# marella/ctransformers

Measured on NVIDIA H100. Metric: decode tokens/s Llama-2-7B Q4_K_M b=1, higher is better.
Workload: dtype int8 (q4_K/q6_K weights x q8_K activations, mma.sync u8 x s8 -> exact int32), fp32 combine in the reference's order

## Files before the change

ctransformers_b200/csrc/engine.cu:

```cuda
#include "engine.cuh"

#include <algorithm>
#include <chrono>
#include <cstdio>
#include <cstring>
#include <stdexcept>

#include "attention.cuh"
#include "matvec.cuh"
#include "prefill.cuh"
#include "repack.cuh"
#include "sample_gpu.cuh"
#include "score_gpu.cuh"
#include "stream.cuh"
#include "tables.hpp"
#include "tp_nccl.hpp"

namespace ctb {

#define CTB_CUDA(expr)                                                                                         \
  do {                                                                                                         \
    cudaError_t e__ = (expr);                                                                                  \
    if (e__ != cudaSuccess)                                                                                    \
      throw std::runtime_error(std::string("CUDA error: ") + cudaGetErrorString(e__) + " at " + __FILE__ + ":" + \
// ... 467 lines not shown
  };
  auto take_input = [&](MVParams& p) {
    if (!xchg_due) return;
    p.x = (const float*)xc_ll_[tp_.rank]; p.x_mode = 2; p.x_parts = tp_.world; p.x_stride = n_embd; p.sum_out = x_sum_into;
  };
  auto mark_exchange = [&](size_t first_op) {
    if (!xchg_due) return;
    if (ops_.size() != first_op + 1) throw std::runtime_error("tensor parallel (fused exchange): the consumer of an exchange must be one mat-vec phase");
    fill_xc(ops_[first_op].ph.xc, 1);
    n_xchg++;
    xchg_due = false; x_sum_into = nullptr;
  };
  const float kq_scale = 1.0f / sqrtf((float)n_embd / (float)hp_.n_head);
  ops_.clear();
  {
    StepOp op{};
    op.ph.kind = PH_EMBED;
    op.ph.em.table = tok_embd_; op.ph.em.row_bytes = tok_row_bytes_; op.ph.em.tokens = d_state_; op.ph.em.out = xa_;
    op.ph.em.type = tok_type_; op.ph.em.K = n_embd; op.ph.em.n_vocab = hp_.n_vocab;
    ops_.push_back(op);
  }
  float* x = xa_;
  float* y = xb_;
  for (int il = 0; il < hp_.n_layer; il++) {
    const LayerW& L = layers_[il];
    uint16_t* kc = kc_ + (size_t)il * hp_.n_ctx * n_kv * k_stride(hd);
    uint16_t* vc = vc_ + (size_t)il * gqa * kv_ctx_pad(hp_.n_ctx);
    AttnParams ap{};
    ap.kc = kc; ap.vc = vc; ap.out = attn_; ap.exp_tab = exp_tab_; ap.state = d_state_; ap.kq_scale = kq_scale;
    ap.n_head = nh_; ap.n_kv = n_kv; ap.hd = hd; ap.n_ctx = hp_.n_ctx; ap.rope = rope_; ap.neox = hp_.falcon ? 1 : 0;
    auto push_attn = [&]() {
      StepOp op{};
      op.ph.kind = PH_ATTN;
      op.ph.at = ap;
      ops_.push_back(op);
    };

    if (!hp_.falcon) {
      float* q = qkv_; float* k = qkv_ + qw; float* v = qkv_ + qw + gqa;
      {
        MVParams p{};
        p.x = x; p.norm_w = L.attn_norm; p.norm_mode = NORM_RMS; p.eps = hp_.eps; p.K = n_embd;
        const size_t first_op = ops_.size();
        take_input(p);
        const DevMat* ws[3] = {&L.wq, &L.wk, &L.wv};
        float* outs[3] = {q, k, v};
        bool done[3] = {false, false, false};
        ap.q = q; ap.k = k; ap.v = v; ap.q_stride = qw; ap.kv_stride = gqa;
        for (int i = 0; i < 3; i++) {
          if (done[i]) continue;
          p.act = act_format_for(ws[i]->type); p.nseg = 0;
          for (int j = i; j < 3; j++)
            if (!done[j] && act_format_for(ws[j]->type) == p.act) { p.seg[p.nseg++] = seg(*ws[j], outs[j]); done[j] = true; }
          push_matvec(p, MVK_QKV);
        }
        mark_exchange(first_op);
      }
      push_attn();
      {
        MVParams p{};
        p.x = attn_; p.norm_mode = NORM_NONE; p.K = qw; p.act = act_format_for(L.wo.type); p.nseg = 1;
        p.seg[0] = (!tp || tp_lead) ? seg(L.wo, y, EPI_ADD, x) : seg(L.wo, y);
        push_matvec(p, MVK_WO);
        if (tp) push_xchg(y);
      }
      {
        MVParams p{};
        p.x = y; p.norm_w = L.ffn_norm; p.norm_mode = NORM_RMS; p.eps = hp_.eps; p.K = n_embd;
        const size_t first_op = ops_.size();
        take_input(p);
        p.act = act_format_for(L.w1.type); p.nseg = 2;
        p.seg[0] = seg(L.w1, ffn_, EPI_SILU); p.seg[1] = seg(L.w3, ffn2_);
        push_matvec(p, MVK_UP);
        mark_exchange(first_op);
      }
      {
        MVParams p{};
        p.x = ffn_; p.x2 = ffn2_; p.x_mode = 1; p.norm_mode = NORM_NONE; p.K = nff_; p.act = act_format_for(L.w2.type); p.nseg = 1;
        p.seg[0] = (!tp || tp_lead) ? seg(L.w2, x, EPI_ADD, y) : seg(L.w2, x);
        push_matvec(p, MVK_DOWN);
        if (tp) push_xchg(x);
      }
    } else {
      const int qkv_w = (hp_.n_head + 2 * n_kv) * hd;
      float* q = qkv_; float* k = qkv_ + (size_t)hp_.n_head * hd; float* v = k + (size_t)n_kv * hd;
      const bool two_norms = L.attn_norm2 != nullptr;
      const bool fuse = !two_norms && act_format_for(L.wqkv.type) == act_format_for(L.w3.type);
      {
        MVParams p{};
        p.x = x; p.norm_mode = NORM_LAYER; p.eps = hp_.eps; p.K = n_embd;
        p.norm_w = two_norms ? L.attn_norm2 : L.attn_norm; p.norm_b = two_norms ? L.attn_norm2_b : L.attn_norm_b;
        p.act = act_format_for(L.wqkv.type); p.nseg = 1;
        p.seg[0] = seg(L.wqkv, qkv_);
        if (fuse) { p.seg[1] = seg(L.w3, ffn_, EPI_GELU); p.nseg = 2; }
        ap.q = q; ap.k = k; ap.v = v; ap.q_stride = qkv_w; ap.kv_stride = qkv_w;
        push_matvec(p, MVK_QKV);
      }
      if (!fuse) {
        MVParams p{};
        p.x = x; p.norm_mode = NORM_LAYER; p.eps = hp_.eps; p.K = n_embd; p.norm_w = L.attn_norm; p.norm_b = L.attn_norm_b;
        p.act = act_format_for(L.w3.type); p.nseg = 1;
        p.seg[0] = seg(L.w3, ffn_, EPI_GELU);
        push_matvec(p, MVK_UP);
      }
      push_attn();
      {
        MVParams p{};
        p.x = attn_; p.norm_mode = NORM_NONE; p.K = n_embd; p.act = act_format_for(L.wo.type); p.nseg = 1;
        p.seg[0] = seg(L.wo, attn_o_);
        push_matvec(p, MVK_WO);
      }
      {
        MVParams p{};
        p.x = ffn_; p.norm_mode = NORM_NONE; p.K = hp_.n_ff; p.act = act_format_for(L.w2.type); p.nseg = 1;
        p.seg[0] = seg(L.w2, y, EPI_ADD2, attn_o_, x);
        push_matvec(p, MVK_DOWN);
      }
      std::swap(x, y);
    }
  }
  n_body_ = (int)ops_.size();
  {
    MVParams p{};
    p.x = x; p.norm_w = out_norm_; p.norm_b = out_norm_b_; p.norm_mode = hp_.falcon ? NORM_LAYER : NORM_RMS; p.eps = hp_.eps; p.K = n_embd;
    const size_t first_op = ops_.size();
    take_input(p);
    p.norm_out = d_embd_; p.act = act_format_for(output_.type); p.nseg = 1;
    p.seg[0] = seg(output_, d_logits_);
    push_matvec(p, MVK_OUT);
    mark_exchange(first_op);

  }
  {
    StepOp op{};
    op.ph.kind = PH_PICK;
    op.ph.pk.logits = d_logits_; op.ph.pk.state = d_state_; op.ph.pk.out_tokens = nullptr; op.ph.pk.n = hp_.n_vocab;
    ops_.push_back(op);
  }
  bool any_stream = false;
  for (const StepOp& op : ops_) any_stream |= op.ph.kind == PH_MATVEC && op.stream;
  std::vector<Phase> phs;
  for (const StepOp& op : ops_) if (op.ph.kind != PH_XCHG && (op.ph.kind != PH_MATVEC || op.stream)) phs.push_back(op.ph);
  const StepLaunch sl = step_launch_shape(phs.data(), (int)phs.size(), sm_count_, max_dyn_smem(k_step<true, false, false>));
  step_grid_ = sl.grid; step_slots_ = sl.n_slots; step_smem_ = sl.smem; step_q3_ = sl.q3;
  if (const char* e = getenv("CTB_ST_SLOTS")) {
    const int want = atoi(e);
    if (want >= ST_W && want < step_slots_ && want % ST_W == 0) { step_smem_ -= (size_t)(step_slots_ - want) * ST_SLOT; step_slots_ = want; }
  }
  ring_attn_ = st_attn_ring_ok(hp_.n_ctx, step_slots_) && !getenv("CTB_NO_RING_ATTN");
  for (StepOp& op : ops_) if (op.ph.kind == PH_ATTN) op.ph.q6 = ring_attn_ ? 1 : 0;
  if (any_stream && step_slots_ < ST_W) throw std::runtime_error("model rows are too long for the step kernel's shared memory");
  if (any_stream) CTB_CUDA(step_set_smem_limit(step_smem_));
  else fused_ = false;
  d_prog_ = (Phase*)alloc((ops_.size() + 1) * sizeof(Phase), 256);
  d_prog_mv_ = (Phase*)alloc((ops_.size() + 1) * sizeof(Phase), 256);
  d_bounds_ = (int*)alloc((ops_.size() + 1) * (size_t)(sm_count_ + 1) * 4, 256);
  d_bounds_mv_ = (int*)alloc((ops_.size() + 1) * (size_t)(sm_count_ + 1) * 4, 256);
}

void Engine::upload_prog(Phase* dst, int* dst_bounds, const std::vector<StepOp>& ops) {
  std::vector<Phase> phs(ops.size());
  for (size_t i = 0; i < ops.size(); i++) phs[i] = ops[i].ph;
  CTB_CUDA(cudaMemcpy(dst, phs.data(), phs.size() * sizeof(Phase), cudaMemcpyHostToDevice));
  std::vector<Phase> run = phs;
  for (size_t i = 0; i < ops.size(); i++) if (ops[i].ph.kind == PH_XCHG || (ops[i].ph.kind == PH_MATVEC && !ops[i].stream)) run[i].kind = -1;
  const std::vector<int> b = step_bounds(run.data(), (int)run.size(), sm_count_);
  CTB_CUDA(cudaMemcpy(dst_bounds, b.data(), b.size() * 4, cudaMemcpyHostToDevice));
}

struct ProfMark {
  Event ev;
  int kind;
};

long Engine::enqueue_ops(const std::vector<StepOp>& ops, const Phase* d_prog, const int* d_bounds, int n, cudaStream_t st, bool fused,
                         std::vector<ProfMark>* marks) {
  long launches = 0;
  auto mark = [&](int kind) {
    if (!marks) return;
    marks->push_back({Event(cudaEventDefault), kind});
    CTB_CUDA(cudaEventRecord(marks->back().ev, st));
  };
  StepLaunch step_shape_;
  step_shape_.grid = step_grid_; step_shape_.n_slots = step_slots_; step_shape_.smem = step_smem_; step_shape_.gen = !attn_fast_hd(hp_.head_dim());
  step_shape_.q3 = step_q3_;
  auto capable = [&](const StepOp& op) { return op.ph.kind != PH_XCHG && (op.ph.kind != PH_MATVEC || op.stream); };
  int i = 0;
  while (i < n) {
    const StepOp& op = ops[i];
    if (fused && capable(op)) {
      int j = i;
      while (j < n && capable(ops[j])) j++;
      mark(-1);
      CTB_CUDA(launch_step(step_shape_, st, d_prog + i, d_bounds + (size_t)i * (sm_count_ + 1), j - i, d_sync_, false, nullptr, tp_peer_));
      launches++;
      mark(0);
      i = j;
      continue;
    }
    mark(-1);
    switch (op.ph.kind) {
      case PH_EMBED:
        k_embed<<<1, 256, 0, st>>>(op.ph.em);
        launches++;
        mark(3);
        break;
      case PH_ATTN:
        CTB_CUDA(launch_kernel(attn_kernel(hp_.head_dim()), dim3(nh_, 1, attn_groups(hp_.head_dim())), dim3(ATTN_THREADS), attn_smem_bytes(hp_.n_ctx, hp_.head_dim()), st, pdl_, op.ph.at));
        launches++;
        mark(1);
        break;
      case PH_XCHG:
        tp_all_reduce(op.ph.em.out, op.ph.em.K, st);
        mark(3);
        break;
      case PH_PICK:
        k_argmax<<<1, ARGMAX_THREADS, 0, st>>>(d_logits_, hp_.n_vocab, d_state_ + 4);
        k_advance<<<1, 1, 0, st>>>(d_state_, d_tokens_out_.as<int>());
        launches += 2;
        mark(3);
        break;
      default:
        if (op.stream) {
          CTB_CUDA(launch_step(step_shape_, st, d_prog + i, d_bounds + (size_t)i * (sm_count_ + 1), 1, d_sync_));
        } else {
          const MVLaunch L = matvec_launch_shape(op.ph.mv, sm_count_);
          CTB_CUDA(launch_matvec_kernel(L, st, op.ph.mv, pdl_));
        }
        launches++;
        mark(0);
    }
    i++;
  }
  CTB_CUDA(cudaGetLastError());
  return launches;
}

int Engine::profile_step(int token, int n_past, double ms_by_kind[4], int count_by_kind[4]) {
  DeviceGuard dev_guard(device_);
  if (tp_.world > 1) throw std::runtime_error("not available in tensor-parallel mode (every rank must run the same launches)");
  drop_lookahead();
  put_step(token, n_past, n_past + 1);
  std::vector<ProfMark> marks;
  enqueue_ops(ops_, d_prog_, d_bounds_, n_body_ + 1, stream_, false, &marks);
  CTB_CUDA(cudaStreamSynchronize(stream_));
  int n = 0;
  for (size_t i = 1; i < marks.size(); i++) {
    float ms = 0;
    cudaEventElapsedTime(&ms, marks[i - 1].ev, marks[i].ev);
    const int k = marks[i].kind;
    if (k >= 0 && k < 4) { ms_by_kind[k] += ms; count_by_kind[k]++; n++; }
  }
  return n;
}

double Engine::time_matvec_only(int reps, long* launches, unsigned mask) {
  if (!mask) mask = ~0u;
  if (tp_.world > 1) throw std::runtime_error("not available in tensor-parallel mode (every rank must run the same launches)");
  drop_lookahead();
  DeviceGuard dev_guard(device_);
  std::vector<StepOp> sel;
  for (int i = 0; i <= n_body_; i++)
    if (ops_[i].ph.kind == PH_MATVEC && ((mask >> ops_[i].mvk) & 1)) sel.push_back(ops_[i]);
  if (sel.empty()) { if (launches) *launches = 0; return 0.0; }
  upload_prog(d_prog_mv_, d_bounds_mv_, sel);
  GraphExec ex;
  {
    const Stream cap(cudaStreamNonBlocking);
    cudaGraph_t g;
    CTB_CUDA(cudaStreamBeginCapture(cap, cudaStreamCaptureModeThreadLocal));
    enqueue_ops(sel, d_prog_mv_, d_bounds_mv_, (int)sel.size(), cap, fused_);
    CTB_CUDA(cudaStreamEndCapture(cap, &g));
    ex = GraphExec(g);
    cudaGraphDestroy(g);
  }
  if (launches) *launches = (long)sel.size();
  const Event e0(cudaEventDefault), e1(cudaEventDefault);
  for (int i = 0; i < 3; i++) CTB_CUDA(cudaGraphLaunch(ex, stream_));
  CTB_CUDA(cudaEventRecord(e0, stream_));
  for (int i = 0; i < reps; i++) CTB_CUDA(cudaGraphLaunch(ex, stream_));
  CTB_CUDA(cudaEventRecord(e1, stream_));
  CTB_CUDA(cudaStreamSynchronize(stream_));
  float ms = 0;
  cudaEventElapsedTime(&ms, e0, e1);
  return (double)ms / reps;
}

long Engine::trace_step(int token, int n_past, unsigned long long* out, long cap_words) {
  DeviceGuard dev_guard(device_);
  if (tp_.world > 1) throw std::runtime_error("not available in tensor-parallel mode (every rank must run the same launches)");
  drop_lookahead();
  const int n = n_body_ + 1;
  for (int i = 0; i < n; i++)
    if (ops_[i].ph.kind == PH_MATVEC && !ops_[i].stream) return 0;
  const long need = 2L * n + 8L * n * step_grid_;
  if (need > cap_words) return -need;
  const DevMem buf((size_t)n * step_grid_ * 64);
  CTB_CUDA(cudaMemset(buf.get(), 0, (size_t)n * step_grid_ * 64));
  StepLaunch L;
  L.grid = step_grid_; L.n_slots = step_slots_; L.smem = step_smem_; L.gen = !attn_fast_hd(hp_.head_dim()); L.q3 = step_q3_;
  for (int rep = 0; rep < 3; rep++) {
    put_step(token, n_past, n_past + 1);
    CTB_CUDA(launch_step(L, stream_, d_prog_, d_bounds_, n, d_sync_, false, buf.as<unsigned long long>()));
    CTB_CUDA(cudaStreamSynchronize(stream_));
  }
  for (int i = 0; i < n; i++) { out[2 * i] = (unsigned long long)ops_[i].ph.kind; out[2 * i + 1] = (unsigned long long)ops_[i].mvk; }
  CTB_CUDA(cudaMemcpy(out + 2 * n, buf.get(), (size_t)n * step_grid_ * 64, cudaMemcpyDeviceToHost));
  return n;
}

void Engine::build_graphs() {
  tokens_out_cap_ = std::max(hp_.n_ctx, 4096);
  d_tokens_out_ = DevMem((size_t)tokens_out_cap_ * 4);
  h_tokens_out_ = HostMem((size_t)tokens_out_cap_ * 4);
  const Stream cap(cudaStreamNonBlocking);
  ops_.back().ph.pk.out_tokens = d_tokens_out_.as<int>();
  upload_prog(d_prog_, d_bounds_, ops_);
  long launches = 0;
  auto capture = [&](bool logits, bool greedy) {
    cudaGraph_t g;
    CTB_CUDA(cudaStreamBeginCapture(cap, cudaStreamCaptureModeThreadLocal));
    launches = enqueue_ops(ops_, d_prog_, d_bounds_, n_body_ + (logits || tp_peer_ ? 1 : 0) + (greedy ? 1 : 0), cap, fused_);
    CTB_CUDA(cudaStreamEndCapture(cap, &g));
    GraphExec ex(g);
    cudaGraphDestroy(g);
    return ex;
  };
  graph_nolog_ = capture(false, false);
  graph_greedy_ = capture(true, true);
  graph_full_ = capture(true, false);
  stats.launches = launches;
}

void Engine::after_eval(int next_pos) {
  spec_pending_ = false;
  spec_deferred_ = false;
  spec_pos_ = -1;
  if (!spec_on_ || next_pos >= hp_.n_ctx || next_pos < kv_high_) return;
  k_argmax<<<1, ARGMAX_THREADS, 0, stream_>>>(d_logits_, hp_.n_vocab, d_state_ + 4);
  k_advance<<<1, 1, 0, stream_>>>(d_state_, d_tokens_out_.as<int>());
  CTB_CUDA(cudaMemcpyAsync(h_spec_tok_.get(), d_state_ + 4, 8, cudaMemcpyDeviceToHost, stream_));
  CTB_CUDA(cudaEventRecord(ev_pick_, stream_));
  spec_pos_ = next_pos;
  if (spec_streak_ >= 2) {
    if (sampler_mode_) spec_deferred_ = true;
    else {
      CTB_CUDA(cudaGraphLaunch(graph_full_, stream_));
      spec_pending_ = true;
    }
  }
}

void Engine::drop_lookahead() { spec_pending_ = false; spec_deferred_ = false; spec_pos_ = -1; spec_streak_ = 0; }

void Engine::launch_deferred_spec() {
  if (!spec_deferred_) return;
  spec_deferred_ = false;
  CTB_CUDA(cudaGraphLaunch(graph_full_, stream_));
  spec_pending_ = true;
}

int Engine::greedy_pick() {
  if (spec_pos_ < 0) return -1;
  DeviceGuard dev_guard(device_);
  CTB_CUDA(cudaEventSynchronize(ev_pick_));
  sampler_mode_ = false;
  launch_deferred_spec();
  const int* pick = h_spec_tok_.as<int>();
  return pick[1] == 1 ? pick[0] : -1;
}

void Engine::put_step(int token, int pos, int n_total) {
  CTB_CUDA(step_ring_.put(stream_, 4, [&](int* st) { st[0] = token; st[1] = pos; st[2] = 0; st[3] = n_total; }));
}

void Engine::decode_one(int token, int pos, int n_total, bool with_logits) {
  put_step(token, pos, n_total);
  CTB_CUDA(cudaGraphLaunch(with_logits ? graph_full_ : graph_nolog_, stream_));
  single_steps_++;
}

int Engine::paths(int* out, int cap) {
  const int v[6] = {fused_ ? 1 : 0, fused_ && ring_attn_ ? 1 : 0, step_slots_, ensure_prefill() ? 1 : 0, (int)prefill_launches_, (int)single_steps_};
  const int n = (int)(sizeof(v) / sizeof(v[0]));
  if (cap < n) return -n;
  std::copy(v, v + n, out);
  return n;
}

void Engine::host_views() {
  eager_ = true;
  if (host_fresh_) return;
  DeviceGuard dev_guard(device_);
  CTB_CUDA(cudaMemcpyAsync(h_logits_.get(), kept_logits_, (size_t)hp_.n_vocab * 4, cudaMemcpyDeviceToHost, stream_));
  CTB_CUDA(cudaMemcpyAsync(h_embd_.get(), kept_embd_, (size_t)hp_.n_embd * 4, cudaMemcpyDeviceToHost, stream_));
  CTB_CUDA(cudaStreamSynchronize(stream_));
  host_fresh_ = true;
}

std::vector<float> Engine::logits_copy() {
  std::vector<float> v((size_t)hp_.n_vocab);
  if (host_fresh_) { memcpy(v.data(), h_logits_.get(), v.size() * 4); return v; }
  DeviceGuard dev_guard(device_);
  CTB_CUDA(cudaMemcpyAsync(v.data(), kept_logits_, v.size() * 4, cudaMemcpyDeviceToHost, stream_));
  CTB_CUDA(cudaStreamSynchronize(stream_));
  return v;
}

void Engine::sample_enqueue(const SampleRow* rows, int R, bool picks) {
  const int S = hp_.n_seq;
  if (R < 0 || R > S) throw std::runtime_error("device sampler: " + std::to_string(R) + " rows for " + std::to_string(S) + " slots");
  const size_t picks_b = (size_t)S * 8, outs_b = (size_t)S * sizeof(SampleGpuOut);
  const size_t bytes = picks_b + outs_b + sg_block_ints(S, S * SG_MAX_LAST) * 4;
  uint8_t* d_buf = (uint8_t*)d_sample_.grow(bytes);
  uint8_t* h_buf = (uint8_t*)h_sample_.grow(bytes);
  SampleGpuOut* d_out = (SampleGpuOut*)(d_buf + picks_b);
  int* h_blk = (int*)(h_buf + picks_b + outs_b);
  int* d_blk = (int*)(d_buf + picks_b + outs_b);
  int n_tok = 0;
  for (int r = 0; r < R; r++) {
    if (!sg_accepts(rows[r].n_last, rows[r].k) || rows[r].slot < 0 || rows[r].slot >= S) throw std::runtime_error("device sampler: a row it does not take");
    n_tok += sg_window(rows[r].n_last);
  }
  for (int r = 0; r < R; r++) sg_put(h_blk, R, r, rows[r].slot, rows[r].last, rows[r].n_last, rows[r].penalty, rows[r].k, hp_.n_vocab);
  if (R > 0) {
    CTB_CUDA(cudaMemcpyAsync(d_blk, h_blk, sg_block_ints(R, n_tok) * 4, cudaMemcpyHostToDevice, stream_));
    sg_launch(sg_rows(d_blk, R, kept_logits_, (size_t)hp_.n_vocab, d_out), R, hp_.n_vocab, stream_);
    CTB_CUDA(cudaGetLastError());
  }
  if (picks) CTB_CUDA(cudaMemcpyAsync(d_buf, kept_pick_, picks_b, cudaMemcpyDeviceToDevice, stream_));
  const size_t from = picks ? 0 : picks_b, to = picks_b + (size_t)R * sizeof(SampleGpuOut);
  if (to > from) CTB_CUDA(cudaMemcpyAsync(h_buf + from, d_buf + from, to - from, cudaMemcpyDeviceToHost, stream_));
}

int Engine::topk_candidates(const int* last, int n_last, float penalty, int k, int* ids, float* logits) {
  if (!sg_accepts(n_last, k)) return -1;
  DeviceGuard dev_guard(device_);
  sampler_mode_ = true;
  const SampleRow row{0, last, n_last, penalty, k};
  sample_enqueue(&row, 1, false);
  CTB_CUDA(cudaEventRecord(ev_sample_, stream_));
  launch_deferred_spec();
  CTB_CUDA(cudaEventSynchronize(ev_sample_));
  return sg_take(*(const SampleGpuOut*)(h_sample_.as<uint8_t>() + (size_t)hp_.n_seq * 8), ids, logits);
}

void Engine::finish_eval(int next_pos, bool hit) {
  CTB_CUDA(cudaMemcpyAsync(kept_logits_, d_logits_, (size_t)hp_.n_vocab * 4, cudaMemcpyDeviceToDevice, stream_));
  CTB_CUDA(cudaMemcpyAsync(kept_embd_, d_embd_, (size_t)hp_.n_embd * 4, cudaMemcpyDeviceToDevice, stream_));
  if (eager_) {
    CTB_CUDA(cudaMemcpyAsync(h_logits_.get(), d_logits_, (size_t)hp_.n_vocab * 4, cudaMemcpyDeviceToHost, stream_));
    CTB_CUDA(cudaMemcpyAsync(h_embd_.get(), d_embd_, (size_t)hp_.n_embd * 4, cudaMemcpyDeviceToHost, stream_));
  }
// ... 519 lines not shown
```

ctransformers_b200/csrc/engine.cuh:

```cuda
#pragma once
#include <cmath>
#include <memory>
#include <string>
#include <vector>

#include "cuda_owned.cuh"
#include "device_types.cuh"
#include "gguf.hpp"

namespace ctb {

struct TPShard {
  int rank = 0, world = 1;
  int head0 = 0, head1 = 0, kv0 = 0, kv1 = 0, ff0 = 0, ff1 = 0;
  void* comm = nullptr;
};
TPShard tp_shard(int n_embd, int n_head, int n_head_kv, int n_ff, int rank, int world);

struct HParams {
  bool falcon = false;
  int n_vocab = 0, n_ctx_train = 0, n_embd = 0, n_ff = 0, n_head = 0, n_head_kv = 0, n_layer = 0, n_rot = 0;
  float eps = 1e-5f, rope_base = 10000.f, rope_scale = 1.f;
  int n_ctx = 512;
  int n_seq = 1;
  bool multi = false;
  int head_dim() const { return n_embd / n_head; }
  int n_embd_gqa() const { return head_dim() * n_head_kv; }
};

struct LayerW {
  DevMat wq, wk, wv, wqkv, wo, w1, w2, w3;
  const float* attn_norm = nullptr; const float* attn_norm_b = nullptr;
  const float* attn_norm2 = nullptr; const float* attn_norm2_b = nullptr;
  const float* ffn_norm = nullptr;
};

struct Phase;
struct StepOp;
struct ProfMark;
struct MVParams;
struct Uploader;
struct PrefillState;

struct MultiTok { int slot, token, pos, n_total; bool last; };
constexpr int MULTI_LAUNCH_TOKENS = 32;

struct SampleRow { int slot; const int* last; int n_last; float penalty; int k; };

struct RowSink {
  float* host = nullptr;
  const int* targets = nullptr;
  double* logprob = nullptr;
  int* greedy = nullptr;
};

struct KvCopy { int src, dst, lo, hi; };

struct EvalStats { double last_eval_ms = 0; long launches = 0; size_t weight_bytes_per_token = 0; long spec_hits = 0; double load_ms = 0; size_t load_bytes = 0; };

class Engine {
 public:
  Engine(const GGUFFile& g, const HParams& hp, int device, const TPShard& tp = TPShard());
  ~Engine();
  Engine(const Engine&) = delete;
  Engine& operator=(const Engine&) = delete;

  void eval_list(const int* tokens, const int* pos, const int* n_total, int n, const RowSink* rows = nullptr);
  void score_kept(int target, double* logprob, int* greedy);
  double decode_greedy(int first_token, int n_past, int n_steps, int* out_tokens);
  double time_matvec_only(int reps, long* launches, unsigned mask = 0);
  int profile_step(int token, int n_past, double ms_by_kind[4], int count_by_kind[4]);
  long trace_step(int token, int n_past, unsigned long long* out, long cap_words);
  std::string multi_refusal();
  void multi_eval(const std::vector<MultiTok>& toks, const std::vector<int>& starts, const RowSink* rows = nullptr);
  void multi_fetch(int slot, float* logits, float* embd);
  const struct SampleGpuOut* multi_sample(const SampleRow* rows, int R, int* picks);
  void multi_reset(int slot);
  long multi_launches() const;
  size_t state_bytes(int n_past, bool results) const;
  int state_k_stride() const;
  void state_save(int slot, int n_past, bool results, void* out);
  void state_load(int slot, int n_past, bool results, const void* in, int last_token);
  void state_fork(int src, const int* dsts, int n);
  size_t kv_reparent(const std::vector<KvCopy>& copies);
  const float* multi_rows(int slot0, int n);
  int paths(int* out, int cap);

  float* logits() { host_views(); return h_logits_.as<float>(); }
  float* embeddings() { host_views(); return h_embd_.as<float>(); }
  bool lazy_logits() const { return !eager_; }
  std::vector<float> logits_copy();
  int topk_candidates(const int* last, int n_last, float penalty, int k, int* ids, float* logits);
  int greedy_pick();
  const HParams& hparams() const { return hp_; }
  EvalStats stats;
  void set_stream(cudaStream_t s);
  cudaStream_t stream() const { return stream_; }

 private:
  Engine(const HParams& hp, int device, const TPShard& tp);
  HParams hp_;
  TPShard tp_;
  int nh_ = 0, nkv_ = 0, nff_ = 0;
  void tp_all_reduce(float* buf, int n, cudaStream_t st);
  bool tp_peer_ = false;
  uint8_t* xc_region_ = nullptr;
  uint2* xc_ll_[8] = {nullptr};
  void tp_setup_peer();
  int device_ = 0;
  Stream stream_;
  DevMem arena_;
  size_t arena_size_ = 0, arena_used_ = 0;
  void* alloc(size_t bytes, size_t align = 256);

  DevMat output_;
  const uint8_t* tok_embd_ = nullptr; int tok_type_ = 0; size_t tok_row_bytes_ = 0;
  const float* out_norm_ = nullptr; const float* out_norm_b_ = nullptr;
  std::vector<LayerW> layers_;
  uint16_t *silu_tab_ = nullptr, *gelu_tab_ = nullptr, *exp_tab_ = nullptr;
  float2* rope_ = nullptr;
  uint16_t *kc_ = nullptr, *vc_ = nullptr;
  int* d_state_ = nullptr;
  float *xa_ = nullptr, *xb_ = nullptr, *qkv_ = nullptr, *attn_ = nullptr, *attn_o_ = nullptr, *ffn_ = nullptr, *ffn2_ = nullptr, *d_logits_ = nullptr, *d_embd_ = nullptr;
  float *kept_logits_ = nullptr, *kept_embd_ = nullptr;
  int* kept_pick_ = nullptr;
  float* kept_logits(int slot) const { return kept_logits_ + (size_t)slot * hp_.n_vocab; }
  float* kept_embd(int slot) const { return kept_embd_ + (size_t)slot * hp_.n_embd; }
  HostMem h_logits_, h_embd_;
  StateRing step_ring_;
  void put_step(int token, int pos, int n_total);
  HostMem h_tokens_out_;
  DevMem d_tokens_out_;
  int tokens_out_cap_ = 0;

  Event ev0_, ev1_, ev_pick_;
  bool spec_on_ = true, spec_pending_ = false;
  bool spec_deferred_ = false;
  bool sampler_mode_ = false;
  Event ev_sample_;
  void launch_deferred_spec();
  int spec_pos_ = -1, spec_streak_ = 0;
  void drop_lookahead();
  int kv_high_ = 0;
  HostMem h_spec_tok_;
  HostMem h_dbg_;
  void after_eval(int next_pos);
  int sm_count_ = 132;

  void init(const GGUFFile& g);
  DevMat upload_matrix(const GGUFTensor& t, struct Uploader& up, int want_K, int want_M, int row0 = 0, int row1 = -1, int k0 = 0, int k1 = -1);
  const float* upload_vector(const GGUFFile& g, const std::string& name, bool required, int want_n);
  std::vector<StepOp> ops_;
  int n_body_ = 0;
  Phase* d_prog_ = nullptr;
  Phase* d_prog_mv_ = nullptr;
  int *d_bounds_ = nullptr, *d_bounds_mv_ = nullptr;
  unsigned* d_sync_ = nullptr;
  int step_grid_ = 0, step_slots_ = 0;
  size_t step_smem_ = 0;
  bool fused_ = true;
  bool step_q3_ = false;
  bool ring_attn_ = false;
  void build_ops();
  void push_matvec(struct MVParams& p, int kind);
  void upload_prog(Phase* dst, int* dst_bounds, const std::vector<StepOp>& ops);
  long enqueue_ops(const std::vector<StepOp>& ops, const Phase* d_prog, const int* d_bounds, int n, cudaStream_t st, bool fused,
                   std::vector<ProfMark>* marks = nullptr);
  void build_graphs();
  bool eager_ = false;
  bool host_fresh_ = true;
  void host_views();
  DevMem d_sample_;
  HostMem h_sample_;
  void sample_enqueue(const SampleRow* rows, int R, bool picks);
  std::unique_ptr<PrefillState> pf_;
  bool multi_ready();
  void need_multi();
  bool prefill_on_ = true;
  int prefill_min_ = 4;
  long prefill_launches_ = 0;
  long single_steps_ = 0;
  bool ensure_prefill();
  void prefill_batch(const int* tokens, const int* pos, const int* n_total, int n, bool last, bool rows = false);
  void launch_batch(const MultiTok* toks, int n, bool whole);
  const RowSink* sink_ = nullptr;
  DevMem d_rows_;
  int rows_pending_ = 0, rows_done_ = 0;
  int rows_n_ = 0;
  DevMem d_score_;
  HostMem h_score_;
  int score_cap_ = 0;
  double* d_lp_ = nullptr;
  int *d_tgt_ = nullptr, *d_gr_ = nullptr;
  struct SinkGuard { Engine* e; ~SinkGuard() { e->sink_ = nullptr; } };
  SinkGuard rows_begin(const RowSink* rows, int n);
  void rows_finish();
  void rows_take(const float* src, int m);
  void rows_push(const float* row);
  void rows_drain();
  void rows_end();
  void decode_one(int token, int pos, int n_total, bool with_logits);
  void head_from(const float* row);
  void finish_eval(int next_pos, bool hit);
  enum : int { MVK_QKV = 0, MVK_WO = 1, MVK_UP = 2, MVK_DOWN = 3, MVK_OUT = 4 };
  bool pdl_ = true;
  HostMem h_stage_;
  DevMem d_copies_;
  HostMem h_copies_;
  void kv_slot_elems(size_t& k, size_t& v) const;
  void zero_slot(int slot);
  void copy_results(int src, int dst);
  GraphExec graph_full_, graph_nolog_, graph_greedy_;
};

size_t engine_arena_bytes(const GGUFFile& g, const HParams& hp);

}
```

ctransformers_b200/csrc/matvec.cuh:

```cuda
#pragma once
#include "device_types.cuh"
#include "attention.cuh"

namespace ctb {

#ifndef CTB_THREADS
#define CTB_THREADS 512
#endif
constexpr int MV_THREADS = CTB_THREADS;
constexpr int MV_WARPS = MV_THREADS / 32;
constexpr int MV_ROWS = 4;
constexpr int MV_MAX_SEG = 3;

enum : int { NORM_NONE = 0, NORM_RMS = 1, NORM_LAYER = 2 };
enum : int { EPI_STORE = 0, EPI_ADD = 1, EPI_GELU = 2, EPI_ADD2 = 3, EPI_SILU = 4 };

#ifndef ST_WATCHDOG_NS
#define ST_WATCHDOG_NS 4000000000ull
#endif
#ifndef XC_WATCHDOG_NS
#define XC_WATCHDOG_NS 30000000000ull
#endif
enum WaitCode : int {
  W_GRID_BARRIER = 1, W_FOLD_FLAG, W_FREE_WEIGHT_SLOT, W_WEIGHT_ITEM, W_FREE_K_SLOT, W_FREE_V_SLOT, W_K_ITEM, W_V_ITEM, W_XCHG,
  W_PF_GRID_BARRIER, W_PF_FREE_SLOT, W_PF_WEIGHT_ITEM, W_CODES
};
constexpr const char* WAIT_TEXT[] = {"?", "grid barrier (aux = phase)", "fold hand-off flag (aux = chunk)", "producer: free weight slot (aux = item)",
                                     "consumer: weight item (aux = item)", "producer: free K slot (attention)", "producer: free V slot (attention)",
                                     "consumer: K item (attention)", "consumer: V item (attention)", "tensor-parallel exchange: a peer's element (aux = exchange number)",
                                     "prefill grid barrier (aux = phase)", "prefill producer: free slot (aux = item)", "prefill consumer: weight item (aux = item)"};
static_assert(sizeof(WAIT_TEXT) / sizeof(WAIT_TEXT[0]) == W_CODES, "one text per wait code");

static __device__ int* g_st_dbg = nullptr;
static __device__ __noinline__ void st_fail(WaitCode code, int aux) {
  int* d = g_st_dbg;
  if (d) { d[0] = code; d[1] = (int)blockIdx.x; d[2] = aux; d[3] = (int)threadIdx.x; __threadfence_system(); }
  __trap();
}
template <typename Done>
__device__ __forceinline__ void bounded_wait(Done&& done, WaitCode code, int aux, unsigned long long limit_ns = ST_WATCHDOG_NS) {
  if (done()) return;
  const unsigned long long t0 = globaltimer_ns();
  while (!done())
    if (globaltimer_ns() - t0 > limit_ns) st_fail(code, aux);
}

struct MVSeg {
  DevMat w;
  float* out;
  const float* res;
  const float* res2;
  int epi;
};

struct MVParams {
  const float* x;
  const float* x2;
  int x_mode;
  int x_parts, x_stride;
  float* sum_out;
  const float* norm_w;
  const float* norm_b;
  float* norm_out;
  float eps;
  int norm_mode;
  int K;
  int act;
  int nseg;
  MVSeg seg[MV_MAX_SEG];
  const uint16_t* silu_tab;
  const uint16_t* gelu_tab;
};

struct ActView {
  const int8_t* qs;
  const float* d;
  const int16_t* bs;
};

__host__ __device__ inline size_t act_smem_bytes(int act, int K) {
  switch (act) {
    case ACT_Q8_K: return (size_t)K + (((size_t)(K / 256) * 4 + 15) & ~(size_t)15) + (size_t)(K / 16) * 2 + 16;
    case ACT_Q8_0: return (size_t)K + (size_t)(K / 32) * 4 + 16;
    case ACT_Q8_1: return (size_t)K + (size_t)(K / 32) * 8 + 16;
    case ACT_F16: return (size_t)K * 2;
    default: return (size_t)K * 4;
  }
}

__host__ __device__ inline size_t q8k_d_bytes(int K) { return ((size_t)(K / 256) * 4 + 15) & ~(size_t)15; }

__device__ __forceinline__ ActView act_view(int act, int K, uint8_t* smem) {
  ActView a;
  a.qs = (const int8_t*)smem;
  const size_t off = ((size_t)K + 15) & ~(size_t)15;
  a.d = (const float*)(smem + off);
  a.bs = (const int16_t*)(smem + off + q8k_d_bytes(K));
  return a;
}

__device__ __forceinline__ int q8k_word_offset(int b, int s, int l) { return ((b * 2 + (s >> 2)) * 8 + l) * 16 + (s & 3) * 4; }


template <bool CG = false>
__device__ __forceinline__ void load16(const float* p, int valid, float (&v)[16]) {
  if (valid >= 16) {
    float4 a, b, c, d;
    if (CG) { a = __ldcg((const float4*)p); b = __ldcg((const float4*)p + 1); c = __ldcg((const float4*)p + 2); d = __ldcg((const float4*)p + 3); }
    else { a = __ldg((const float4*)p); b = __ldg((const float4*)p + 1); c = __ldg((const float4*)p + 2); d = __ldg((const float4*)p + 3); }
    v[0] = a.x; v[1] = a.y; v[2] = a.z; v[3] = a.w; v[4] = b.x; v[5] = b.y; v[6] = b.z; v[7] = b.w;
    v[8] = c.x; v[9] = c.y; v[10] = c.z; v[11] = c.w; v[12] = d.x; v[13] = d.y; v[14] = d.z; v[15] = d.w;
  } else {
#pragma unroll
    for (int e = 0; e < 16; e++) v[e] = e < valid ? (CG ? __ldcg(p + e) : __ldg(p + e)) : 0.f;
  }
}

template <int NT, int BAR>
__device__ __forceinline__ double block_sum_f64(double s, double* red ) {
  s = warp_sum(s);
  bar_sync<BAR, NT>();
  if ((threadIdx.x & 31) == 0) red[threadIdx.x >> 5] = s;
  bar_sync<BAR, NT>();
  double t = 0.0;
#pragma unroll
  for (int w = 0; w < NT / 32; w++) t += red[w];
  return t;
}
template <int NT, int BAR>
__device__ __forceinline__ void block_sum2_max_f64(double& s, double& a, double& g, double* red) {
  constexpr int NW = NT / 32;
#pragma unroll
  for (int o = 16; o > 0; o >>= 1) {
    s += __shfl_xor_sync(0xffffffffu, s, o);
    a += __shfl_xor_sync(0xffffffffu, a, o);
    g = fmax(g, __shfl_xor_sync(0xffffffffu, g, o));
  }
  bar_sync<BAR, NT>();
  if ((threadIdx.x & 31) == 0) { red[threadIdx.x >> 5] = s; red[NW + (threadIdx.x >> 5)] = a; red[2 * NW + (threadIdx.x >> 5)] = g; }
  bar_sync<BAR, NT>();
  s = 0.0;
  a = 0.0;
#pragma unroll
  for (int w = 0; w < NW; w++) { s += red[w]; a += red[NW + w]; g = fmax(g, red[2 * NW + w]); }
}

__device__ __forceinline__ uint32_t pack4(const int* q) {
  return (uint32_t)(q[0] & 0xff) | ((uint32_t)(q[1] & 0xff) << 8) | ((uint32_t)(q[2] & 0xff) << 16) | ((uint32_t)(q[3] & 0xff) << 24);
}

__device__ __forceinline__ void load16_ll(const uint2* p, unsigned epoch, float (&u)[16]) {
  uint4 q[8];
  bounded_wait([&] {
    bool ok = true;
#pragma unroll
    for (int j = 0; j < 8; j++) {
      asm volatile("ld.volatile.global.v4.u32 {%0,%1,%2,%3}, [%4];" : "=r"(q[j].x), "=r"(q[j].y), "=r"(q[j].z), "=r"(q[j].w) : "l"(p + 2 * j) : "memory");
    }
#pragma unroll
    for (int j = 0; j < 8; j++) ok &= q[j].y == epoch && q[j].w == epoch;
    return ok;
  }, W_XCHG, (int)epoch, XC_WATCHDOG_NS);
#pragma unroll
  for (int j = 0; j < 8; j++) { u[2 * j] = __uint_as_float(q[j].x); u[2 * j + 1] = __uint_as_float(q[j].z); }
}

template <bool XC = false>
__device__ __forceinline__ void load16x(const MVParams& xs, int base, int valid, float (&v)[16], unsigned epoch = 0) {
  if (XC && xs.x_mode == 2) {
    if (valid <= 0) {
#pragma unroll
      for (int e = 0; e < 16; e++) v[e] = 0.f;
      return;
    }
    const uint2* ll = (const uint2*)xs.x + (size_t)(epoch & 1u) * xs.x_parts * xs.x_stride;
    load16_ll(ll + base, epoch, v);
    for (int r = 1; r < xs.x_parts; r++) {
      float u[16];
      load16_ll(ll + (size_t)r * xs.x_stride + base, epoch, u);
#pragma unroll
      for (int e = 0; e < 16; e++) v[e] = __fadd_rn(v[e], u[e]);
    }
    return;
  }
  load16<true>(xs.x + base, valid, v);
  if (xs.x_mode == 1) {
    float u[16];
    load16<true>(xs.x2 + base, valid, u);
#pragma unroll
    for (int e = 0; e < 16; e++) v[e] = __fmul_rn(v[e], u[e]);
  }
}

struct NormPre { float w0[16], bias0[16]; };
__device__ __forceinline__ void preload_norm(NormPre& np, const MVParams& p) {
  const int t = threadIdx.x;
  if (p.norm_mode != NORM_NONE && p.norm_w) load16(p.norm_w + t * 16, p.K - t * 16, np.w0);
  if (p.norm_mode != NORM_NONE && p.norm_b) load16(p.norm_b + t * 16, p.K - t * 16, np.bias0);
}

__device__ __forceinline__ unsigned min_exp(unsigned emin, float t) {
  const unsigned bits = __float_as_uint(t) & 0x7fffffffu;
  return bits ? min(emin, max(bits >> 23, 1u)) : emin;
}
__device__ __forceinline__ double lsb_inv(unsigned emin) { return ldexp(1.0, 150 - (int)emin); }

enum : int { NORM_TERM_SQ = 0, NORM_TERM_X = 1, NORM_TERM_DEV = 2 };
template <bool XC>
static __device__ __noinline__ double seq_sum_warp0(const float* x, const float* x2, int x_mode, int x_parts, int x_stride, int K, int kind,
                                                    float mean, unsigned epoch) {
  MVParams xs;
  xs.x = x; xs.x2 = x2; xs.x_mode = x_mode; xs.x_parts = x_parts; xs.x_stride = x_stride;
  const int lane = threadIdx.x & 31;
  double seq = 0.0;
  for (int base = 0; base < K; base += 512) {
    float v[16];
    load16x<XC>(xs, base + lane * 16, K - base - lane * 16, v, epoch);
    for (int l = 0; l < 32; l++)
#pragma unroll
      for (int i = 0; i < 16; i++) {
        float t = __shfl_sync(0xffffffffu, v[i], l);
        if (kind == NORM_TERM_DEV) t = __fsub_rn(t, mean);
        if (base + l * 16 + i < K) seq += kind == NORM_TERM_X ? (double)t : (double)__fmul_rn(t, t);
      }
  }
  return seq;
}

template <int NT, int BAR, bool XC>
__device__ __forceinline__ float norm_stat(double s, double a, double g, bool a_is_s, int kind, float mean, const MVParams& xs, double* red,
                                           unsigned epoch) {
  const int K = xs.K;
  if (a_is_s) a = s = block_sum_f64<NT, BAR>(s, red);
  else block_sum2_max_f64<NT, BAR>(s, a, g, red);
  if (!isfinite(s) || (!a_is_s && __dmul_ru(a, g) < 0x1p52)) return (float)(s / (double)K);
  const double e = __dmul_ru(a, (double)K * 0x1.0000001p-52);
  const float lo = (float)(__dsub_rd(s, e) / (double)K), hi = (float)(__dadd_ru(s, e) / (double)K);
  if (lo == hi) return lo;
  const double seq = threadIdx.x < 32 ? seq_sum_warp0<XC>(xs.x, xs.x2, xs.x_mode, xs.x_parts, xs.x_stride, K, kind, mean, epoch) : 0.0;
  bar_sync<BAR, NT>();
  if (threadIdx.x == 0) red[0] = seq;
  bar_sync<BAR, NT>();
  return (float)(red[0] / (double)K);
}

template <int NT, int BAR, bool XC = false>
__device__ __forceinline__ void stage_activation(const MVParams& xs, const NormPre& np, int act, uint8_t* smem, double* red, bool write_norm, unsigned epoch = 0) {
  const float* nw = xs.norm_w;
  const float* nb_ = xs.norm_b;
  float* norm_out = xs.norm_out;
  const int norm_mode = xs.norm_mode, K = xs.K;
  const float eps = xs.eps;
  const int t = threadIdx.x, lane = t & 31;
  const int passes = (K + NT * 16 - 1) / (NT * 16);
  float mean = 0.f, scale = 1.f;
  float v0[16];
  load16x<XC>(xs, t * 16, K - t * 16, v0, epoch);
  if (norm_mode == NORM_RMS) {
    double ss = 0.0;
    for (int ps = 0; ps < passes; ps++) {
      const int base = (ps * NT + t) * 16;
      if ((base & ~511) >= K) continue;
      float v[16];
      if (ps == 0) {
#pragma unroll
        for (int e = 0; e < 16; e++) v[e] = v0[e];
      } else load16x<XC>(xs, base, K - base, v, epoch);
#pragma unroll
      for (int e = 0; e < 16; e++) ss += (double)__fmul_rn(v[e], v[e]);
    }
    const float m = norm_stat<NT, BAR, XC>(ss, ss, 0.0, true, NORM_TERM_SQ, 0.f, xs, red, epoch);
    scale = __fdiv_rn(1.0f, __fsqrt_rn(__fadd_rn(m, eps)));
  } else if (norm_mode == NORM_LAYER) {
    double s1 = 0.0, a1 = 0.0;
    unsigned emin = 255;
    for (int ps = 0; ps < passes; ps++) {
      const int base = (ps * NT + t) * 16;
      if ((base & ~511) >= K) continue;
      float v[16];
      load16x<XC>(xs, base, K - base, v, epoch);
#pragma unroll
      for (int e = 0; e < 16; e++) {
        s1 += (double)v[e];
        a1 += (double)fabsf(v[e]);
        emin = min_exp(emin, v[e]);
      }
    }
    mean = norm_stat<NT, BAR, XC>(s1, a1, lsb_inv(emin), false, NORM_TERM_X, 0.f, xs, red, epoch);
    double s2 = 0.0;
    for (int ps = 0; ps < passes; ps++) {
      const int base = (ps * NT + t) * 16;
      if ((base & ~511) >= K) continue;
      float v[16];
      load16x<XC>(xs, base, K - base, v, epoch);
#pragma unroll
      for (int e = 0; e < 16; e++) { const float d = (base + e < K) ? __fsub_rn(v[e], mean) : 0.f; s2 += (double)__fmul_rn(d, d); }
    }
    const float var = norm_stat<NT, BAR, XC>(s2, s2, 0.0, true, NORM_TERM_DEV, mean, xs, red, epoch);
    scale = __fdiv_rn(1.0f, __fsqrt_rn(__fadd_rn(var, eps)));
  }
  int8_t* qs = (int8_t*)smem;
  const size_t off = ((size_t)K + 15) & ~(size_t)15;
  float* dd = (float*)(smem + off);
  int16_t* bs = (int16_t*)(smem + off + q8k_d_bytes(K));
  for (int ps = 0; ps < passes; ps++) {
    const int base = (ps * NT + t) * 16;
    const int valid = K - base;
    if ((base & ~511) >= K) continue;
    float v[16];
    if (ps == 0) {
#pragma unroll
      for (int e = 0; e < 16; e++) v[e] = v0[e];
    } else load16x<XC>(xs, base, valid, v, epoch);
    if (XC && write_norm && xs.x_mode == 2 && xs.sum_out && valid > 0) {
#pragma unroll
      for (int e = 0; e < 16; e++) if (e < valid) xs.sum_out[base + e] = v[e];
    }
    if (norm_mode != NORM_NONE) {
      float w[16], bb[16];
      if (ps == 0) {
#pragma unroll
        for (int e = 0; e < 16; e++) { w[e] = np.w0[e]; bb[e] = np.bias0[e]; }
      } else {
        if (nw) load16(nw + base, valid, w);
        if (nb_) load16(nb_ + base, valid, bb);
      }
#pragma unroll
      for (int e = 0; e < 16; e++) {
        float y = v[e];
        if (norm_mode == NORM_LAYER) y = __fsub_rn(y, mean);
        y = __fmul_rn(y, scale);
        if (nw) y = __fmul_rn(y, w[e]);
        if (nb_) y = __fadd_rn(y, bb[e]);
        v[e] = y;
      }
    }
    if (write_norm && norm_out && valid > 0) {
#pragma unroll
      for (int e = 0; e < 16; e++) if (e < valid) norm_out[base + e] = v[e];
    }
    if (act == ACT_Q8_K) {
      float amax = 0.f, mx = 0.f;
#pragma unroll
      for (int e = 0; e < 16; e++) { const float ax = fabsf(v[e]); if (ax > amax) { amax = ax; mx = v[e]; } }
      float gmax = amax;
#pragma unroll
      for (int o = 8; o > 0; o >>= 1) gmax = fmaxf(gmax, __shfl_xor_sync(0xffffffffu, gmax, o));
      const unsigned who = __ballot_sync(0xffffffffu, amax == gmax);
      const int hbase = lane & 16, hl = lane & 15;
      const unsigned mine = (who >> hbase) & 0xffffu;
      const float maxv = __shfl_sync(0xffffffffu, mx, hbase + __ffs(mine) - 1);
      if (valid > 0) {
        const int b = base >> 8;
        int q[16];
        int sum = 0;
        if (gmax == 0.f) {
#pragma unroll
          for (int e = 0; e < 16; e++) q[e] = 0;
          if (hl == 0) dd[b] = 0.f;
        } else {
          const float iscale = __fdiv_rn(-128.f, maxv);
#pragma unroll
          for (int e = 0; e < 16; e++) {
            const float val = __fmaf_rn(iscale, v[e], 12582912.f);
            q[e] = min(127, (__float_as_int(val) & 0x007fffff) - 0x00400000);
            sum += q[e];
          }
          if (hl == 0) dd[b] = __fdiv_rn(1.f, iscale);
        }
        bs[b * 16 + hl] = (int16_t)sum;
#pragma unroll
        for (int j = 0; j < 4; j++) {
          const int wi = hl * 4 + j;
          *(uint32_t*)(qs + q8k_word_offset(b, wi >> 3, wi & 7)) = pack4(q + 4 * j);
        }
      }
    } else if (act == ACT_Q8_0) {
      float amax = 0.f;
#pragma unroll
      for (int e = 0; e < 16; e++) amax = fmaxf(amax, fabsf(v[e]));
      amax = fmaxf(amax, __shfl_xor_sync(0xffffffffu, amax, 1));
      if (valid > 0) {
        const float d = __fdiv_rn(amax, 127.f);
        const float id = amax != 0.f ? __fdiv_rn(127.f, amax) : 0.f;
        int q[16];
#pragma unroll
        for (int e = 0; e < 16; e++) q[e] = __float2int_rn(__fmul_rn(v[e], id));
        *(uint4*)(qs + base) = make_uint4(pack4(q), pack4(q + 4), pack4(q + 8), pack4(q + 12));
        if ((lane & 1) == 0) dd[base >> 5] = h2f(f2h(d));
      }
    } else if (act == ACT_Q8_1) {
      float amax = 0.f;
#pragma unroll
      for (int e = 0; e < 16; e++) amax = fmaxf(amax, fabsf(v[e]));
      amax = fmaxf(amax, __shfl_xor_sync(0xffffffffu, amax, 1));
      const float d = __fdiv_rn(amax, 127.f);
      const float id = amax != 0.f ? __fdiv_rn(127.f, amax) : 0.f;
      int q[16];
      int sum = 0;
#pragma unroll
      for (int e = 0; e < 16; e++) { q[e] = __float2int_rn(__fmul_rn(v[e], id)); sum += q[e]; }
      sum += __shfl_xor_sync(0xffffffffu, sum, 1);
      if (valid > 0) {
        *(uint4*)(qs + base) = make_uint4(pack4(q), pack4(q + 4), pack4(q + 8), pack4(q + 12));
        if ((lane & 1) == 0) *(float2*)(dd + (base >> 4)) = make_float2(d, __fmul_rn(d, (float)sum));
      }
    } else if (act == ACT_F16) {
      uint16_t* h = (uint16_t*)smem;
#pragma unroll
      for (int e = 0; e < 16; e++) if (e < valid) h[base + e] = f2h(v[e]);
    } else {
      float* f = (float*)smem;
#pragma unroll
      for (int e = 0; e < 16; e++) if (e < valid) f[base + e] = v[e];
    }
  }
  bar_sync<BAR, NT>();
}

__device__ __forceinline__ float group_hsum8(float v) {
  v = v + __shfl_xor_sync(0xffffffffu, v, 4);
  v = v + __shfl_xor_sync(0xffffffffu, v, 2);
  v = v + __shfl_xor_sync(0xffffffffu, v, 1);
  return v;
}

__device__ __forceinline__ float dot_q40(const DevMat& w, int row, const ActView& a, int l) {
  const int nb = w.nb;
  const uint8_t* qrow = w.qs + (size_t)row * nb * 16 + (l & 3) * 4;
  const uint16_t* drow = w.d + (size_t)row * nb;
  const int shift = (l >> 2) * 4;
  float acc = 0.f;
#pragma unroll 8
  for (int b = 0; b < nb; b++) {
    const uint32_t q = (uint32_t)__ldg((const int*)(qrow + (size_t)b * 16));
    const float dw = h2f(__ldg(drow + b));
    const int aw = *(const int*)(a.qs + b * 32 + l * 4);
    const float yd = a.d[b];
    const uint32_t nib = (q >> shift) & 0x0f0f0f0fu;
    const uint32_t bx = ((nib | 0x80808080u) - 0x08080808u) ^ 0x80808080u;
    acc = __fmaf_rn(__fmul_rn(dw, yd), (float)__dp4a((int)bx, aw, 0), acc);
  }
  return group_hsum8(acc);
}

__device__ __forceinline__ float dot_q50(const DevMat& w, int row, const ActView& a, int l) {
  const int nb = w.nb;
  const uint8_t* qrow = w.qs + (size_t)row * nb * 16 + (l & 3) * 4;
  const uint32_t* hrow = (const uint32_t*)w.qh + (size_t)row * nb;
  const uint16_t* drow = w.d + (size_t)row * nb;
  const int shift = (l >> 2) * 4;
  float acc = 0.f;
#pragma unroll 8
  for (int b = 0; b < nb; b++) {
    const uint32_t q = (uint32_t)__ldg((const int*)(qrow + (size_t)b * 16));
    const uint32_t h4 = (__ldg(hrow + b) >> (4 * l)) & 0xfu;
    const float dw = h2f(__ldg(drow + b));
    const int aw = *(const int*)(a.qs + b * 32 + l * 4);
    const float yd = a.d[b];
    const uint32_t nib = (q >> shift) & 0x0f0f0f0fu;
    const uint32_t set = (h4 * 0x00204081u) & 0x01010101u;
    const uint32_t bx = nib | ((set ^ 0x01010101u) * 0xf0u);
    acc = __fmaf_rn(__fmul_rn(dw, yd), (float)__dp4a((int)bx, aw, 0), acc);
  }
  return group_hsum8(acc);
}

__device__ __forceinline__ float dot_q80(const DevMat& w, int row, const ActView& a, int l) {
  const int nb = w.nb;
  const uint8_t* qrow = w.qs + (size_t)row * nb * 32 + l * 4;
  const uint16_t* drow = w.d + (size_t)row * nb;
  float acc = 0.f;
#pragma unroll 8
  for (int b = 0; b < nb; b++) {
    const int q = __ldg((const int*)(qrow + (size_t)b * 32));
    const float dw = h2f(__ldg(drow + b));
    const int aw = *(const int*)(a.qs + b * 32 + l * 4);
    acc = __fmaf_rn(__fmul_rn(dw, a.d[b]), (float)__dp4a(q, aw, 0), acc);
  }
  return group_hsum8(acc);
}

template <bool Q5>
__device__ __forceinline__ float dot_q1(const DevMat& w, int row, const ActView& a, int l) {
  const int nb = w.nb;
  const uint8_t* qrow = w.qs + (size_t)row * nb * 16 + (l & 3) * 4;
  const uint32_t* hrow = (const uint32_t*)w.qh + (size_t)row * nb;
  const uint16_t* drow = w.d + (size_t)row * nb;
  const uint16_t* mrow = w.mn + (size_t)row * nb;
  const int shift = (l >> 2) * 4;
  float acc = 0.f, summs = 0.f;
#pragma unroll 8
  for (int b = 0; b < nb; b++) {
    const uint32_t q = (uint32_t)__ldg((const int*)(qrow + (size_t)b * 16));
    const float dw = h2f(__ldg(drow + b));
    const float mw = h2f(__ldg(mrow + b));
    const int aw = *(const int*)(a.qs + b * 32 + l * 4);
    const float2 ds = *(const float2*)(a.d + 2 * b);
    uint32_t bx = (q >> shift) & 0x0f0f0f0fu;
    if (Q5) bx |= ((((__ldg(hrow + b) >> (4 * l)) & 0xfu) * 0x00204081u) & 0x01010101u) << 4;
    acc = __fmaf_rn(__fmul_rn(dw, ds.x), (float)__dp4a((int)bx, aw, 0), acc);
    summs = __fmaf_rn(mw, ds.y, summs);
  }
  return __fadd_rn(group_hsum8(acc), summs);
}

__device__ __forceinline__ float dot_legacy(const DevMat& w, int row, const ActView& a, int l) {
  switch (w.type) {
    case GT_Q4_0: return dot_q40(w, row, a, l);
    case GT_Q5_0: return dot_q50(w, row, a, l);
    case GT_Q4_1: return dot_q1<false>(w, row, a, l);
    case GT_Q5_1: return dot_q1<true>(w, row, a, l);
    default: return dot_q80(w, row, a, l);
  }
}

__device__ __forceinline__ float warp_reduce_f32x8(float v) {
  v = v + __shfl_xor_sync(0xffffffffu, v, 16);
  v = v + __shfl_xor_sync(0xffffffffu, v, 8);
  v = v + __shfl_xor_sync(0xffffffffu, v, 4);
  v = v + __shfl_xor_sync(0xffffffffu, v, 1);
  v = v + __shfl_xor_sync(0xffffffffu, v, 2);
  return v;
}

__device__ __forceinline__ float dot_f16_row(const DevMat& w, int row, const uint8_t* smem, int lane) {
  const uint16_t* xa = (const uint16_t*)smem;
  const uint16_t* wr = (const uint16_t*)w.qs + (size_t)row * w.K;
  const int np = w.K & ~31;
// ... 82 lines not shown
```

ctransformers_b200/csrc/ops_abi.cu:

```cuda
#include <cmath>
#include <cstdio>
#include <cstring>
#include <ctime>
#include <functional>
#include <stdexcept>
#include <string>
#include <vector>

#include "../../include/ctransformers_b200.h"
#include "attention.cuh"
#include "cuda_owned.cuh"
#include "matvec.cuh"
#include "prefill.cuh"
#include "repack.cuh"
#include "sample_gpu.cuh"
#include "sampler.hpp"
#include "score_gpu.cuh"
#include "stream.cuh"
#include "tables.hpp"

using namespace ctb;

namespace {

// ... 432 lines not shown
        Phase ph{};
        ph.kind = PH_ATTN; ph.q6 = 1; ph.at = ap;
        const StepLaunch L = step_launch_shape(&ph, 1, sm_count(), max_dyn_smem(k_step<true, false, false>));
        if (!st_attn_ring_ok(n_ctx, L.n_slots)) throw std::runtime_error("the step kernel's ring cannot carry K / V at this n_ctx");
      }
      const size_t smem = attn_smem_bytes(n_ctx, hd);
      if (path == 0) OPS_CUDA(cudaFuncSetAttribute(attn_kernel(hd), cudaFuncAttributeMaxDynamicSharedMemorySize, (int)std::max<size_t>(smem, 48 * 1024)));
      for (int i = 0; i < n_tok; i++) {
        AttnParams a = ap;
        a.q += (size_t)i * nq; a.k += (size_t)i * nkv; a.v += (size_t)i * nkv; a.out += (size_t)i * nq; a.state += (size_t)i * 4;
        if (path == 0) {
          attn_kernel(hd)<<<dim3(n_head, 1, attn_groups(hd)), ATTN_THREADS, smem>>>(a);
          OPS_CUDA(cudaGetLastError());
        } else {
          Phase ph{};
          ph.kind = PH_ATTN; ph.q6 = path == 1 ? 1 : 0; ph.at = a;
          run_phases({ph});
        }
      }
    }
    OPS_CUDA(cudaDeviceSynchronize());
    OPS_CUDA(cudaMemcpy(out, dout.get(), nq * n_tok * 4, cudaMemcpyDeviceToHost));
    OPS_CUDA(cudaMemcpy(kp.data(), dkc.get(), kp.size() * 2, cudaMemcpyDeviceToHost));
    OPS_CUDA(cudaMemcpy(vp.data(), dvc.get(), vp.size() * 2, cudaMemcpyDeviceToHost));
    kv_from_device(kp, vp, n_kv, hd, n_ctx, kcache, vcache);
  });
}

int ctb_prefill_mul_mat(int nseg, const int* types, const void* const* w_blocks, const int* rows, int K, int n_tok, const float* x,
                        const float* x2, int norm_mode, const float* norm_w, const float* norm_b, float eps, const int* epi,
                        const float* res, const float* res2, float* out, int n_ctx, int head_dim, int* n_slots) {
  return guarded("ctb_prefill_mul_mat", [&] {
    if (nseg < 1 || nseg > MV_MAX_SEG) throw std::runtime_error("1 to 3 segments");
    if (K < 256 || K % 256) throw std::runtime_error("K must be a positive multiple of 256");
    if (n_tok < 1) throw std::runtime_error("n_tok must be at least 1");
    if (norm_mode < NORM_NONE || norm_mode > NORM_LAYER || (x2 && norm_mode != NORM_NONE)) throw std::runtime_error("norm mode 0, 1 or 2, and 0 with x2");
    if ((norm_mode != NORM_NONE && !norm_w) || (norm_mode == NORM_LAYER && !norm_b)) throw std::runtime_error("RMSNorm needs norm_w, LayerNorm norm_w and norm_b");
    if (norm_mode == NORM_NONE) norm_w = nullptr;
    if (norm_mode != NORM_LAYER) norm_b = nullptr;
    if (!attn_head_dim_ok(head_dim)) throw std::runtime_error("head_dim must be even, from 32 to 256");
    if (n_ctx < 1) throw std::runtime_error("n_ctx must be at least 1");
    int off[MV_MAX_SEG + 1] = {0};
    for (int s = 0; s < nseg; s++) {
      if (!type_is_kquant(types[s])) throw std::runtime_error("the batched kernel takes K-quant weights only");
      if (rows[s] < 1) throw std::runtime_error("every segment needs at least one row");
      if (epi[s] < EPI_STORE || epi[s] > EPI_SILU) throw std::runtime_error("unknown epilogue");
      if ((epi[s] == EPI_ADD || epi[s] == EPI_ADD2) && !res) throw std::runtime_error("ADD / ADD2 need res");
      if (epi[s] == EPI_ADD2 && !res2) throw std::runtime_error("ADD2 needs res2");
      off[s + 1] = off[s] + rows[s];
    }
    const int W = off[nseg];
    int slots = 0;
    size_t smem = 0;
    if (!pstep_shape(pb_work_bytes(K, n_ctx, head_dim), slots, smem)) throw std::runtime_error("no batched prefill at this n_ctx: its attention scratch does not fit");
    std::vector<DevMem> keep;
    DevMat mats[MV_MAX_SEG];
    for (int s = 0; s < nseg; s++) mats[s] = upload(keep, types[s], w_blocks[s], K, rows[s]);
    DevMem dx((size_t)PB_T * K * 4), dx2((size_t)PB_T * K * 4), dout((size_t)PB_T * W * 4), dres((size_t)PB_T * W * 4), dres2((size_t)PB_T * W * 4),
        dnw((size_t)K * 4), dnb((size_t)K * 4), dq(pb_qbuf_bytes(K)), dst((PB_T * 4 + 4) * 4);
    OPS_CUDA(cudaMemset(dq.get(), 0, pb_qbuf_bytes(K)));
    OPS_CUDA(cudaMemset(dout.get(), 0, (size_t)PB_T * W * 4));
    if (norm_w) OPS_CUDA(cudaMemcpy(dnw.get(), norm_w, (size_t)K * 4, cudaMemcpyHostToDevice));
    if (norm_b) OPS_CUDA(cudaMemcpy(dnb.get(), norm_b, (size_t)K * 4, cudaMemcpyHostToDevice));
    MVParams m{};
    m.x = dx.as<float>(); m.x2 = x2 ? dx2.as<float>() : nullptr; m.x_mode = x2 ? 1 : 0;
    m.norm_w = norm_w ? dnw.as<float>() : nullptr; m.norm_b = norm_b ? dnb.as<float>() : nullptr; m.norm_mode = norm_mode; m.eps = eps;
    m.K = K; m.act = ACT_Q8_K; m.nseg = nseg; m.silu_tab = tables().silu; m.gelu_tab = tables().gelu;
    for (int s = 0; s < nseg; s++) {
      m.seg[s].w = mats[s]; m.seg[s].out = dout.as<float>() + off[s]; m.seg[s].epi = epi[s];
      if (epi[s] == EPI_ADD || epi[s] == EPI_ADD2) m.seg[s].res = dres.as<float>() + off[s];
      if (epi[s] == EPI_ADD2) m.seg[s].res2 = dres2.as<float>() + off[s];
    }
    struct Rows { const float* p; int ld; };
    const Rows bufs[5] = {{dx.as<float>(), K}, {dx2.as<float>(), K}, {dout.as<float>(), W}, {dres.as<float>(), W}, {dres2.as<float>(), W}};
    auto bat = [&](const float* p, int& ld) -> float* {
      ld = 0;
      if (!p) return nullptr;
      for (const Rows& b : bufs)
        if (p >= b.p && p < b.p + (size_t)PB_T * b.ld) { ld = b.ld; return const_cast<float*>(p); }
      throw std::runtime_error("pointer outside the token buffers");
    };
    std::vector<PPhase> prog;
    pb_matvec_phases(m, dq.as<uint8_t>(), dst.as<int>(), bat, prog);
    DevMem dprog((prog.size() + 1) * sizeof(PPhase));
    OPS_CUDA(cudaMemcpy(dprog.get(), prog.data(), prog.size() * sizeof(PPhase), cudaMemcpyHostToDevice));
    OPS_CUDA(pstep_set_smem_limit(smem));
    for (int b = 0; b < n_tok; b += PB_T) {
      const int n = std::min(PB_T, n_tok - b);
      std::vector<int> st(PB_T * 4 + 4, 0);
      for (int i = 0; i < PB_T; i++) {
        const int k = std::min(i, n - 1);
        st[i * 4 + 1] = b + k; st[i * 4 + 3] = b + k + 1;
      }
      st[PB_T * 4] = n;
      OPS_CUDA(cudaMemcpy(dst.get(), st.data(), st.size() * 4, cudaMemcpyHostToDevice));
      OPS_CUDA(cudaMemcpy(dx.get(), x + (size_t)b * K, (size_t)n * K * 4, cudaMemcpyHostToDevice));
      if (x2) OPS_CUDA(cudaMemcpy(dx2.get(), x2 + (size_t)b * K, (size_t)n * K * 4, cudaMemcpyHostToDevice));
      if (res) OPS_CUDA(cudaMemcpy(dres.get(), res + (size_t)b * W, (size_t)n * W * 4, cudaMemcpyHostToDevice));
      if (res2) OPS_CUDA(cudaMemcpy(dres2.get(), res2 + (size_t)b * W, (size_t)n * W * 4, cudaMemcpyHostToDevice));
      OPS_CUDA(launch_pstep(sm_count(), slots, smem, 0, dprog.as<PPhase>(), (int)prog.size(), sync_words(), pstep_q3(prog)));
      OPS_CUDA(cudaDeviceSynchronize());
      OPS_CUDA(cudaMemcpy(out + (size_t)b * W, dout.get(), (size_t)n * W * 4, cudaMemcpyDeviceToHost));
    }
    if (n_slots) *n_slots = slots;
  });
}

int ctb_ffn_gate(int type, const void* w1_blocks, const void* w3_blocks, const float* x, float* out, int K, int M) {
  return guarded("ctb_ffn_gate", [&] {
    std::vector<DevMem> keep;
    const DevMat w1 = upload(keep, type, w1_blocks, K, M), w3 = upload(keep, type, w3_blocks, K, M);
    DevMem dx((size_t)K * 4), dg((size_t)M * 4), du((size_t)M * 4), dy((size_t)M * 4);
    OPS_CUDA(cudaMemcpy(dx.get(), x, (size_t)K * 4, cudaMemcpyHostToDevice));
    MVParams p{};
    p.x = dx.as<float>(); p.norm_mode = NORM_NONE; p.K = K; p.act = act_format_for(type); p.nseg = 2;
    p.seg[0].w = w1; p.seg[0].out = dg.as<float>(); p.seg[0].epi = EPI_SILU; p.seg[1].w = w3; p.seg[1].out = du.as<float>();
    run_matvec(p);
    const size_t smem = (size_t)M * 4 + 64;
    OPS_CUDA(cudaFuncSetAttribute(k_gate_dump, cudaFuncAttributeMaxDynamicSharedMemorySize, (int)std::max<size_t>(smem, 48 * 1024)));
    MVParams q{};
    q.x = dg.as<float>(); q.x2 = du.as<float>(); q.x_mode = 1; q.norm_mode = NORM_NONE; q.K = M;
    k_gate_dump<<<1, MV_THREADS, smem>>>(q, dy.as<float>());
    OPS_CUDA(cudaGetLastError());
    OPS_CUDA(cudaMemcpy(out, dy.get(), (size_t)M * 4, cudaMemcpyDeviceToHost));
  });
}

int ctb_matvec_partition(const int* types, const int* rows, int nseg, int K, int n_sm, int* first_tile, int* meta) {
  if (nseg < 1 || nseg > MV_MAX_SEG || K <= 0 || K % 256 != 0 || n_sm < 1) return -1;
  MVParams p{};
  p.K = K; p.nseg = nseg; p.act = ACT_Q8_K;
  for (int s = 0; s < nseg; s++) {
    if (!type_is_kquant(types[s]) || rows[s] < 1) return -1;
    p.seg[s].w.type = types[s]; p.seg[s].w.K = K; p.seg[s].w.M = rows[s]; p.seg[s].w.nb = K / 256;
  }
  TileSpace ts;
  ts.init(p);
  const int nb = K / 256;
  long max_items = 0;
  for (int c = 0; c <= n_sm; c++) first_tile[c] = ts.boundary(c, n_sm);
  for (int c = 0; c < n_sm; c++) {
    long items = 0;
    for (int tile = first_tile[c]; tile < first_tile[c + 1]; tile++) {
      int tl = tile;
      items += st_chunks(types[ts.locate(tl)], nb);
    }
    max_items = std::max(max_items, items);
  }
  meta[0] = n_sm; meta[1] = ST_SLOT; meta[2] = ST_MAXT; meta[3] = ts.ntiles; meta[4] = ST_W; meta[5] = ST_ROWS; meta[6] = (int)max_items;
  meta[7] = st_chunk_blocks(GT_Q4_K) | (st_chunk_blocks(GT_Q5_K) << 8) | (st_chunk_blocks(GT_Q6_K) << 16) | (st_chunk_blocks(GT_Q3_K) << 24);
  return 0;
}

int ctb_get_row(int type, const void* table_blocks, int K, int n_rows, int row, float* out) {
  return guarded("ctb_get_row", [&] {
    const size_t rb = raw_row_bytes(type, K);
    DevMem dt(rb * n_rows), dtok(4), dout((size_t)K * 4);
    OPS_CUDA(cudaMemcpy(dt.get(), table_blocks, rb * n_rows, cudaMemcpyHostToDevice));
    OPS_CUDA(cudaMemcpy(dtok.get(), &row, 4, cudaMemcpyHostToDevice));
    EmbedParams em{};
    em.table = dt.as<uint8_t>(); em.row_bytes = rb; em.tokens = dtok.as<int>(); em.out = dout.as<float>(); em.type = type; em.K = K; em.n_vocab = n_rows;
    k_embed<<<1, 256>>>(em);
    OPS_CUDA(cudaGetLastError());
    OPS_CUDA(cudaMemcpy(out, dout.get(), (size_t)K * 4, cudaMemcpyDeviceToHost));
  });
}

int ctb_argmax_path(int path, const float* logits, int n, int* out) {
  return guarded("ctb_argmax_path", [&] {
    if (path < 0 || path > 1) throw std::runtime_error("unknown argmax path " + std::to_string(path));
    if (n < 1) throw std::runtime_error("no logits");
    DevMem dlog((size_t)n * 4);
    OPS_CUDA(cudaMemcpy(dlog.get(), logits, (size_t)n * 4, cudaMemcpyHostToDevice));
    if (path == 0) {
      argmax_on_device(dlog.as<float>(), n, out);
      return;
    }
    const int step = out[2];
    if (step < 0 || step >= (1 << 20)) throw std::runtime_error("step out of range");
    DevMem dstate(5 * 4), dtok((size_t)(step + 1) * 4);
    OPS_CUDA(cudaMemcpy(dstate.get(), out, 5 * 4, cudaMemcpyHostToDevice));
    OPS_CUDA(cudaMemset(dtok.get(), 0xff, (size_t)(step + 1) * 4));
    Phase ph{};
    ph.kind = PH_PICK;
    ph.pk.logits = dlog.as<float>(); ph.pk.state = dstate.as<int>(); ph.pk.out_tokens = dtok.as<int>(); ph.pk.n = n;
    run_phases({ph});
    OPS_CUDA(cudaMemcpy(out, dstate.get(), 5 * 4, cudaMemcpyDeviceToHost));
    OPS_CUDA(cudaMemcpy(out + 5, dtok.as<int>() + step, 4, cudaMemcpyDeviceToHost));
  });
}

int ctb_sample_topk(const float* logits, int n, const int* last_tokens, int n_last, float repetition_penalty, int k, int* ids, float* lg) {
  int count = -1;
  const int rc = guarded("ctb_sample_topk", [&] {
    if (n < 1 || !sg_accepts(n_last, k)) throw std::runtime_error("n < 1, or a window or k the device sampler does not take");
    DevMem dlog((size_t)n * 4);
    OPS_CUDA(cudaMemcpy(dlog.get(), logits, (size_t)n * 4, cudaMemcpyHostToDevice));
    const SampleGpuOut o = topk_on_device(dlog.as<float>(), n, last_tokens, n_last, repetition_penalty, k);
    if (o.nan) { count = -2; return; }
    count = o.count;
    for (int i = 0; i < std::min(o.count, SG_MAX_OUT); i++) { ids[i] = o.id[i]; lg[i] = o.logit[i]; }
  });
  return rc == 0 ? count : -1;
}

int ctb_sample_device(const float* logits, int n, const int* last_tokens, int n_last, int top_k, float top_p, float temperature,
                      float repetition_penalty, int seed, int* used_device) {
  int tok = -1;
  const int rc = guarded("ctb_sample_device", [&] {
    if (n < 1) throw std::runtime_error("no logits");
    if (seed < 0) seed = (int)time(nullptr);
    std::mt19937 rng((unsigned)seed);
    DevMem dlog((size_t)n * 4);
    OPS_CUDA(cudaMemcpy(dlog.get(), logits, (size_t)n * 4, cudaMemcpyHostToDevice));
    bool dev = false;
    tok = sample_lazy(
        n, last_tokens, n_last, top_k, top_p, temperature, repetition_penalty, rng, dev,
        [&] {
          int pk[2];
          argmax_on_device(dlog.as<float>(), n, pk);
          return pk[1] == 1 ? pk[0] : -1;
        },
        [&](const int* last, int nl, float pen, int k, int* i, float* l) {
          if (!sg_accepts(nl, k)) return -1;
          return sg_take(topk_on_device(dlog.as<float>(), n, last, nl, pen, k), i, l);
        },
        [&] { return std::vector<float>(logits, logits + n); });
    *used_device = dev ? 1 : 0;
  });
  return rc == 0 ? tok : -1;
}

int ctb_sample_topk_rows(const float* logits, int n_rows, int n, const int* last_off, const int* last_tokens, const float* repetition_penalty,
                         const int* k, int* count, int* ids, float* lg) {
  return guarded("ctb_sample_topk_rows", [&] {
    check_rows(n_rows, n, last_off, last_tokens);
    std::vector<int> rows;
    for (int r = 0; r < n_rows; r++) {
      count[r] = -1;
      if (sg_accepts(last_off[r + 1] - last_off[r], k[r])) rows.push_back(r);
    }
    DevMem dlog((size_t)n_rows * n * 4);
    OPS_CUDA(cudaMemcpy(dlog.get(), logits, (size_t)n_rows * n * 4, cudaMemcpyHostToDevice));
    const std::vector<SampleGpuOut> o = topk_rows_on_device(dlog.as<float>(), n, rows, last_off, last_tokens, repetition_penalty, k);
    for (size_t i = 0; i < rows.size(); i++) {
      const int r = rows[i];
      count[r] = o[i].nan ? -2 : o[i].count;
      for (int j = 0; !o[i].nan && j < std::min(o[i].count, SG_MAX_OUT); j++) {
        ids[(size_t)r * SG_MAX_OUT + j] = o[i].id[j];
        lg[(size_t)r * SG_MAX_OUT + j] = o[i].logit[j];
      }
    }
  });
}

int ctb_sample_device_rows(const float* logits, int n_rows, int n, const int* last_off, const int* last_tokens, const int* top_k, const float* top_p,
                           const float* temperature, const float* repetition_penalty, const int* seed, int* tokens, int* used_device) {
  return guarded("ctb_sample_device_rows", [&] {
    check_rows(n_rows, n, last_off, last_tokens);
    DevMem dlog((size_t)n_rows * n * 4);
    OPS_CUDA(cudaMemcpy(dlog.get(), logits, (size_t)n_rows * n * 4, cudaMemcpyHostToDevice));
    std::vector<int> picks((size_t)2 * n_rows), rows, row_of(n_rows, -1);
    for (int r = 0; r < n_rows; r++) {
      argmax_on_device(dlog.as<float>() + (size_t)r * n, n, &picks[2 * r]);
      const int nl = last_off[r + 1] - last_off[r];
      if (sample_is_greedy(top_k[r], repetition_penalty[r], nl) || !sg_accepts(nl, top_k[r])) continue;
      row_of[r] = (int)rows.size();
      rows.push_back(r);
    }
    const std::vector<SampleGpuOut> o = topk_rows_on_device(dlog.as<float>(), n, rows, last_off, last_tokens, repetition_penalty, top_k);
    for (int r = 0; r < n_rows; r++) {
      std::mt19937 rng((unsigned)(seed[r] < 0 ? (int)time(nullptr) : seed[r]));
      const float* row = logits + (size_t)r * n;
      bool dev = false;
      tokens[r] = sample_lazy(
          n, last_tokens ? last_tokens + last_off[r] : nullptr, last_off[r + 1] - last_off[r], top_k[r], top_p[r], temperature[r], repetition_penalty[r],
          rng, dev, [&] { return picks[2 * r + 1] == 1 ? picks[2 * r] : -1; },
          [&](const int*, int, float, int, int* i, float* l) { return row_of[r] < 0 ? -1 : sg_take(o[row_of[r]], i, l); },
          [&] { return std::vector<float>(row, row + n); });
      used_device[r] = dev ? 1 : 0;
    }
  });
}

int ctb_row_logprob(const float* rows, int n_rows, int n_vocab, const int* targets, double* logprob, int* greedy) {
  return guarded("ctb_row_logprob", [&] {
    if (n_rows < 1 || n_vocab < 1) throw std::runtime_error("no rows");
    for (int r = 0; r < n_rows; r++)
      if (targets[r] < -1 || targets[r] >= n_vocab) throw std::runtime_error("target " + std::to_string(targets[r]) + " of row " + std::to_string(r) + " is out of range");
    DevMem drows((size_t)n_rows * n_vocab * 4), dt((size_t)n_rows * 4), dlp((size_t)n_rows * 8), dg((size_t)n_rows * 4);
    OPS_CUDA(cudaMemcpy(drows.get(), rows, (size_t)n_rows * n_vocab * 4, cudaMemcpyHostToDevice));
    OPS_CUDA(cudaMemcpy(dt.get(), targets, (size_t)n_rows * 4, cudaMemcpyHostToDevice));
    rl_launch(drows.as<float>(), n_rows, n_vocab, dt.as<int>(), dlp.as<double>(), dg.as<int>(), 0);
    OPS_CUDA(cudaGetLastError());
    OPS_CUDA(cudaMemcpy(logprob, dlp.get(), (size_t)n_rows * 8, cudaMemcpyDeviceToHost));
    OPS_CUDA(cudaMemcpy(greedy, dg.get(), (size_t)n_rows * 4, cudaMemcpyDeviceToHost));
  });
}

}
```

ctransformers_b200/csrc/stream.cuh:

```cuda
#pragma once
#include "matvec.cuh"

namespace ctb {

#ifndef CTB_ST_WARPS
#define CTB_ST_WARPS 10
#endif
constexpr int ST_W = CTB_ST_WARPS;
constexpr int ST_NT = ST_W * 32;
constexpr int ST_THREADS = ST_NT + 32;
constexpr int ST_SLOT = 9216;
#ifndef CTB_ST_DEPTH
#define CTB_ST_DEPTH 2
#endif
constexpr int ST_MAX_DEPTH = CTB_ST_DEPTH;
constexpr int ST_MAX_SLOTS = ST_W * ST_MAX_DEPTH;
constexpr int ST_MAXT = 16;
constexpr int ST_ROWS = 16;
constexpr int ST_BAR = 1;
constexpr int ST_STATE = 6;

#ifndef CTB_CHUNK_Q3
#define CTB_CHUNK_Q3 5
#endif
#ifndef CTB_CHUNK_Q4
#define CTB_CHUNK_Q4 4
#endif
#ifndef CTB_CHUNK_Q5
#define CTB_CHUNK_Q5 3
#endif
#ifndef CTB_CHUNK_Q6
#define CTB_CHUNK_Q6 2
#endif
struct StType { int rb, kb, nm; };
template <bool Q3 = true>
__host__ __device__ constexpr StType st_type(int type) {
  return Q3 && type == GT_Q3_K ? StType{110, CTB_CHUNK_Q3, 0}
                               : (type == GT_Q4_K ? StType{144, CTB_CHUNK_Q4, 2} : (type == GT_Q5_K ? StType{176, CTB_CHUNK_Q5, 1} : StType{210, CTB_CHUNK_Q6, 0}));
}
template <int TYPE> struct StTraits {
  static constexpr int KB = st_type(TYPE).kb, BB = ST_ROWS * st_type(TYPE).rb, NM = st_type(TYPE).nm;
  static_assert(KB * BB <= ST_SLOT, "a work item must fit one ring slot");
};
__host__ __device__ inline int st_row_block_bytes(int type) { return st_type(type).rb; }
template <bool Q3 = true>
__host__ __device__ inline int st_block_bytes(int type) { return ST_ROWS * st_type<Q3>(type).rb; }
template <bool Q3 = true>
__host__ __device__ inline int st_chunk_blocks(int type) { return st_type<Q3>(type).kb; }
template <bool Q3 = true>
__host__ __device__ inline int st_tile_cost(int type) { return st_type<Q3>(type).rb / 2; }
template <bool Q3 = true>
__host__ __device__ inline int st_chunks(int type, int nb) {
  constexpr int K3 = StTraits<GT_Q3_K>::KB, K4 = StTraits<GT_Q4_K>::KB, K5 = StTraits<GT_Q5_K>::KB, K6 = StTraits<GT_Q6_K>::KB;
  if (Q3 && type == GT_Q3_K) return (nb + K3 - 1) / K3;
  return type == GT_Q4_K ? (nb + K4 - 1) / K4 : (type == GT_Q5_K ? (nb + K5 - 1) / K5 : (nb + K6 - 1) / K6);
}
__host__ __device__ inline size_t st_matrix_bytes(int type, int M, int nb) { return (size_t)((M + ST_ROWS - 1) / ST_ROWS) * nb * st_block_bytes(type); }

__device__ __forceinline__ void st_decode(int type, int o, int& rl, int& src) {
  if (type == GT_Q3_K) {
    if (o < 1536) {
      const bool qs = o < 1024;
      const int r = qs ? o : o - 1024, q = qs ? r >> 3 : r >> 2, hr = q >> 5, lane = q & 31, h = hr >> 1, rr = hr & 1, g = lane >> 2, t = lane & 3;
      rl = rr * 8 + g;
      src = (qs ? 32 + ((r >> 2) & 1) * 32 : 0) + 4 * (t + 4 * h) + (r & 3);
      return;
    }
    if (o < 1728) { const int r = o - 1536; rl = r / 12; src = 96 + r % 12; return; }
    rl = (o - 1728) >> 1; src = 108; return;
  }
  const int q4 = (type == GT_Q6_K) ? 0 : (type == GT_Q5_K ? 48 : 16);
  if (o < 2048) {
    const int q = o >> 4, hr = q >> 5, lane = q & 31, h = hr >> 1, rr = hr & 1, g = lane >> 2, t = lane & 3, l = t + 4 * h;
    const int wi = (o >> 2) & 3, byte = o & 3;
    rl = rr * 8 + g;
    src = type == GT_Q6_K ? ((wi >> 1) * 64 + (wi & 1) * 32 + 4 * l + byte) : (q4 + 32 * wi + 4 * l + byte);
    return;
  }
  if (type == GT_Q4_K) { const int r = o - 2048; rl = r >> 4; src = r & 15; return; }
  if (type == GT_Q5_K) {
    if (o < 2560) {
      const int q = (o - 2048) >> 2, hr = q >> 5, lane = q & 31, h = hr >> 1, rr = hr & 1, g = lane >> 2, t = lane & 3;
      rl = rr * 8 + g; src = 16 + 4 * (t + 4 * h) + (o & 3);
      return;
    }
    const int r = o - 2560; rl = r >> 4; src = r & 15; return;
  }
  if (o < 3072) {
    const int r = o - 2048, q = r >> 3, hr = q >> 5, lane = q & 31, h = hr >> 1, rr = hr & 1, g = lane >> 2, t = lane & 3;
    rl = rr * 8 + g; src = 128 + ((r >> 2) & 1) * 32 + 4 * (t + 4 * h) + (r & 3);
    return;
  }
  if (o < 3328) { const int r = o - 3072; rl = r >> 4; src = 192 + (r & 15); return; }
  rl = (o - 3328) >> 1; src = 208;
}

static __global__ void k_repack_stream(int type, const uint8_t* __restrict__ raw, int M, int nb, uint16_t* __restrict__ st) {
  const int rbb = st_row_block_bytes(type), half = rbb * ST_ROWS / 2;
  const size_t n_units = (size_t)((M + ST_ROWS - 1) / ST_ROWS) * nb * half;
  for (size_t idx = (size_t)blockIdx.x * blockDim.x + threadIdx.x; idx < n_units; idx += (size_t)gridDim.x * blockDim.x) {
    const size_t piece = idx / half;
    const int o = (int)(idx % half) * 2;
    const size_t tile = piece / nb;
    const int b = (int)(piece % nb);
    int rl, src;
    st_decode(type, o, rl, src);
    const size_t row = tile * ST_ROWS + rl;
    st[idx] = row < (size_t)M ? *(const uint16_t*)(raw + (row * nb + b) * rbb + src) : (uint16_t)0;
  }
}

struct RingPos { uint32_t slot, parity; };
__device__ __forceinline__ RingPos ring_pos(uint32_t i, uint32_t owner, uint32_t owners, uint32_t depth) { return {(i % depth) * owners + owner, (i / depth) & 1u}; }
__device__ __forceinline__ RingPos st_ring(uint32_t n, uint32_t depth) { return ring_pos(n / ST_W, n % ST_W, ST_W, depth); }

__device__ __forceinline__ uint32_t st_smem(const void* p) { return (uint32_t)__cvta_generic_to_shared(p); }
__device__ __forceinline__ void mbar_init(uint64_t* bar, uint32_t count) { asm volatile("mbarrier.init.shared::cta.b64 [%0], %1;" ::"r"(st_smem(bar)), "r"(count) : "memory"); }
__device__ __forceinline__ void mbar_expect_tx(uint64_t* bar, uint32_t bytes) {
  asm volatile("mbarrier.arrive.expect_tx.shared::cta.b64 _, [%0], %1;" ::"r"(st_smem(bar)), "r"(bytes) : "memory");
}
__device__ __forceinline__ void mbar_arrive(uint64_t* bar) { asm volatile("mbarrier.arrive.shared::cta.b64 _, [%0];" ::"r"(st_smem(bar)) : "memory"); }
__device__ __forceinline__ bool mbar_try_wait(uint64_t* bar, uint32_t parity) {
  uint32_t ok;
  asm volatile("{\n .reg .pred p;\n mbarrier.try_wait.parity.shared::cta.b64 p, [%1], %2;\n selp.u32 %0, 1, 0, p;\n}" : "=r"(ok) : "r"(st_smem(bar)), "r"(parity) : "memory");
  return ok != 0;
}
__device__ __forceinline__ void mbar_wait(uint64_t* bar, uint32_t parity, WaitCode code, int aux) {
  bounded_wait([&] { return mbar_try_wait(bar, parity); }, code, aux);
}
__device__ __forceinline__ void ring_init(uint64_t* full_bar, uint64_t* empty_bar, int n_slots, int consumers_per_slot) {
  if (threadIdx.x == 0) {
    for (int s = 0; s < n_slots; s++) { mbar_init(&full_bar[s], 1); mbar_init(&empty_bar[s], consumers_per_slot); }
    asm volatile("fence.mbarrier_init.release.cluster;" ::: "memory");
  }
  __syncthreads();
}
__device__ __forceinline__ void bulk_g2s(void* dst, const void* src, uint32_t bytes, uint64_t* bar) {
  asm volatile("cp.async.bulk.shared::cluster.global.mbarrier::complete_tx::bytes [%0], [%1], %2, [%3];" ::"r"(st_smem(dst)), "l"(src), "r"(bytes), "r"(st_smem(bar)) : "memory");
}
__device__ __forceinline__ void bulk_g2s_hint(void* dst, const void* src, uint32_t bytes, uint64_t* bar, uint64_t pol) {
  asm volatile("cp.async.bulk.shared::cluster.global.mbarrier::complete_tx::bytes.L2::cache_hint [%0], [%1], %2, [%3], %4;" ::"r"(st_smem(dst)), "l"(src), "r"(bytes),
               "r"(st_smem(bar)), "l"(pol) : "memory");
}
__device__ __forceinline__ uint64_t l2_policy_evict_first() {
  uint64_t p;
  asm volatile("createpolicy.fractional.L2::evict_first.b64 %0, 1.0;" : "=l"(p));
  return p;
}
__device__ __forceinline__ void mma_u8s8(int (&d)[4], uint32_t a0, uint32_t a1, uint32_t a2, uint32_t a3, uint32_t b0, uint32_t b1, int c0, int c1) {
  asm("mma.sync.aligned.m16n8k32.row.col.s32.u8.s8.s32 {%0,%1,%2,%3}, {%4,%5,%6,%7}, {%8,%9}, {%10,%11,%12,%13};"
      : "=r"(d[0]), "=r"(d[1]), "=r"(d[2]), "=r"(d[3])
      : "r"(a0), "r"(a1), "r"(a2), "r"(a3), "r"(b0), "r"(b1), "r"(c0), "r"(c1), "r"(c0), "r"(c1));
}

struct StAct {
  const int8_t* qs;
  const float* d;
  const uint32_t* pairs;
  const int* cneg;
  const int8_t* zero;
  const struct XchgParams* xc;
  unsigned epoch;
};
__host__ __device__ inline size_t st_off_pairs(int K) { return ((((size_t)K + 15) & ~(size_t)15) + q8k_d_bytes(K) + (size_t)(K / 16) * 2 + 15) & ~(size_t)15; }
__host__ __device__ inline size_t st_act_bytes(int K, bool q6) { return st_off_pairs(K) + (size_t)(K / 256) * 16 + (q6 ? (size_t)K : 0) + 256 + 16; }

template <int NT, int BAR>
__device__ __forceinline__ StAct st_act_extras(uint8_t* smem, int K, bool q6) {
  const ActView a = act_view(ACT_Q8_K, K, smem);
  StAct s;
  s.qs = a.qs; s.d = a.d;
  uint32_t* pairs = (uint32_t*)(smem + st_off_pairs(K));
  int* cneg = (int*)(smem + st_off_pairs(K) + (size_t)(K / 256) * 16);
  s.pairs = pairs; s.cneg = cneg;
  const int nb = K >> 8;
  int* zero = (int*)(smem + st_off_pairs(K) + (size_t)nb * 16 + (q6 ? (size_t)K : 0));
  s.zero = (const int8_t*)zero;
  if (threadIdx.x < 64) zero[threadIdx.x] = 0;
  for (int i = threadIdx.x; i < nb * 4; i += NT) {
    const int16_t* b4 = a.bs + (i >> 2) * 16 + 4 * (i & 3);
    const int p0 = (int)b4[0] + (int)b4[1], p1 = (int)b4[2] + (int)b4[3];
    pairs[i] = (uint32_t)(p0 & 0xffff) | ((uint32_t)p1 << 16);
  }
  if (q6) {
    for (int i = threadIdx.x; i < nb * 64; i += NT) {
      const int b = i >> 6, grp = (i >> 3) & 7, l = i & 7;
      const int w = *(const int*)(a.qs + q8k_word_offset(b, grp, l));
      cneg[((b * 4 + (l >> 1)) * 8 + grp) * 2 + (l & 1)] = -32 * __dp4a(0x01010101, w, 0);
    }
  }
  bar_sync<BAR, NT>();
  return s;
}

__device__ __forceinline__ void unpack_k4(uint32_t s0, uint32_t s1, uint32_t s2, uint32_t& sc03, uint32_t& sc47, uint32_t& m03, uint32_t& m47) {
  sc03 = s0 & 0x3f3f3f3fu;
  m03 = s1 & 0x3f3f3f3fu;
  sc47 = (s2 & 0x0f0f0f0fu) | (((s0 >> 6) & 0x03030303u) << 4);
  m47 = ((s2 >> 4) & 0x0f0f0f0fu) | (((s1 >> 6) & 0x03030303u) << 4);
}
__device__ __forceinline__ int pack16(int lo, int hi) { return (int)__byte_perm((uint32_t)lo, (uint32_t)hi, 0x5410); }
__device__ __forceinline__ int scale_fold8(int d0, int d1, int d2, int d3, int d4, int d5, int d6, int d7, uint32_t s03, uint32_t s47) {
  int s = __dp2a_lo(pack16(d0, d1), (int)s03, 0);
  s = __dp2a_hi(pack16(d2, d3), (int)s03, s);
  s = __dp2a_lo(pack16(d4, d5), (int)s47, s);
  s = __dp2a_hi(pack16(d6, d7), (int)s47, s);
  return s;
}

struct Terms { float p[4]; float pm[2]; float dd[2]; float ddm[2]; };

__device__ __forceinline__ void load_b_operands(const StAct& a, int b, int g, int t, uint32_t (&bA)[8], uint32_t (&bB)[8]) {
  const int8_t* word = a.qs + b * 256 + g * 16;
  const int8_t* pa = (g == t) ? word : a.zero;
  const int8_t* pb = (g == t + 4) ? word : a.zero;
  const int4 la = *(const int4*)pa, ha = *(const int4*)(pa + 128), lb = *(const int4*)pb, hb = *(const int4*)(pb + 128);
  bA[0] = la.x; bA[1] = la.y; bA[2] = la.z; bA[3] = la.w; bA[4] = ha.x; bA[5] = ha.y; bA[6] = ha.z; bA[7] = ha.w;
  bB[0] = lb.x; bB[1] = lb.y; bB[2] = lb.z; bB[3] = lb.w; bB[4] = hb.x; bB[5] = hb.y; bB[6] = hb.z; bB[7] = hb.w;
}

template <int TYPE>
__device__ __forceinline__ void block_terms(const uint8_t* blk, int b, const StAct& a, int lane, Terms& r);

template <>
__device__ __forceinline__ void block_terms<GT_Q4_K>(const uint8_t* blk, int b, const StAct& a, int lane, Terms& r) {
  const int g = lane >> 2, t = lane & 3;
  const int4* qp = (const int4*)blk;
  const int4 w00 = qp[lane], w01 = qp[32 + lane], w10 = qp[64 + lane], w11 = qp[96 + lane];
  const int4 h0 = ((const int4*)(blk + 2048))[g], h1 = ((const int4*)(blk + 2048))[8 + g];
  uint32_t bA[8], bB[8];
  load_b_operands(a, b, g, t, bA, bB);
  const uint32_t W[4][4] = {{(uint32_t)w00.x, (uint32_t)w01.x, (uint32_t)w10.x, (uint32_t)w11.x}, {(uint32_t)w00.y, (uint32_t)w01.y, (uint32_t)w10.y, (uint32_t)w11.y},
                            {(uint32_t)w00.z, (uint32_t)w01.z, (uint32_t)w10.z, (uint32_t)w11.z}, {(uint32_t)w00.w, (uint32_t)w01.w, (uint32_t)w10.w, (uint32_t)w11.w}};
  int D[8][4];
#pragma unroll
  for (int j = 0; j < 4; j++) {
    mma_u8s8(D[2 * j], W[j][0] & 0x0f0f0f0fu, W[j][1] & 0x0f0f0f0fu, W[j][2] & 0x0f0f0f0fu, W[j][3] & 0x0f0f0f0fu, bA[2 * j], bB[2 * j], 0, 0);
    mma_u8s8(D[2 * j + 1], (W[j][0] >> 4) & 0x0f0f0f0fu, (W[j][1] >> 4) & 0x0f0f0f0fu, (W[j][2] >> 4) & 0x0f0f0f0fu, (W[j][3] >> 4) & 0x0f0f0f0fu, bA[2 * j + 1],
             bB[2 * j + 1], 0, 0);
  }
  const float yd = a.d[b];
  const uint32_t pw = a.pairs[b * 4 + t];
#pragma unroll
  for (int rr = 0; rr < 2; rr++) {
    const int4 h = rr ? h1 : h0;
    uint32_t sc03, sc47, m03, m47;
    unpack_k4((uint32_t)h.y, (uint32_t)h.z, (uint32_t)h.w, sc03, sc47, m03, m47);
#pragma unroll
    for (int c = 0; c < 2; c++) {
      const int i = rr * 2 + c;
      r.p[i] = (float)scale_fold8(D[0][i], D[1][i], D[2][i], D[3][i], D[4][i], D[5][i], D[6][i], D[7][i], sc03, sc47);
    }
    r.dd[rr] = __fmul_rn(yd, h2f((uint16_t)((uint32_t)h.x & 0xffffu)));
    r.ddm[rr] = __fmul_rn(-yd, h2f((uint16_t)((uint32_t)h.x >> 16)));
    const uint32_t mw = (t < 2 ? m03 : m47) >> ((t & 1) * 16);
    r.pm[rr] = (float)__dp2a_lo((int)pw, (int)mw, 0);
  }
}

template <>
__device__ __forceinline__ void block_terms<GT_Q5_K>(const uint8_t* blk, int b, const StAct& a, int lane, Terms& r) {
  const int g = lane >> 2, t = lane & 3;
  const int4* qp = (const int4*)blk;
  const int4 w00 = qp[lane], w01 = qp[32 + lane], w10 = qp[64 + lane], w11 = qp[96 + lane];
  const uint32_t* hp = (const uint32_t*)(blk + 2048);
  const uint32_t HB[4] = {hp[lane], hp[32 + lane], hp[64 + lane], hp[96 + lane]};
  const int4 h0 = ((const int4*)(blk + 2560))[g], h1 = ((const int4*)(blk + 2560))[8 + g];
  uint32_t bA[8], bB[8];
  load_b_operands(a, b, g, t, bA, bB);
  const uint32_t W[4][4] = {{(uint32_t)w00.x, (uint32_t)w01.x, (uint32_t)w10.x, (uint32_t)w11.x}, {(uint32_t)w00.y, (uint32_t)w01.y, (uint32_t)w10.y, (uint32_t)w11.y},
                            {(uint32_t)w00.z, (uint32_t)w01.z, (uint32_t)w10.z, (uint32_t)w11.z}, {(uint32_t)w00.w, (uint32_t)w01.w, (uint32_t)w10.w, (uint32_t)w11.w}};
  int D[8][4];
#pragma unroll
  for (int j = 0; j < 4; j++) {
    uint32_t lo[4], hi[4];
#pragma unroll
    for (int i = 0; i < 4; i++) {
      lo[i] = (W[j][i] & 0x0f0f0f0fu) | (((HB[i] >> (2 * j)) & 0x01010101u) << 4);
      hi[i] = ((W[j][i] >> 4) & 0x0f0f0f0fu) | (((HB[i] >> (2 * j + 1)) & 0x01010101u) << 4);
    }
    mma_u8s8(D[2 * j], lo[0], lo[1], lo[2], lo[3], bA[2 * j], bB[2 * j], 0, 0);
    mma_u8s8(D[2 * j + 1], hi[0], hi[1], hi[2], hi[3], bA[2 * j + 1], bB[2 * j + 1], 0, 0);
  }
  const float yd = a.d[b];
  const uint4 pw = *(const uint4*)(a.pairs + b * 4);
#pragma unroll
  for (int rr = 0; rr < 2; rr++) {
    const int4 h = rr ? h1 : h0;
    uint32_t sc03, sc47, m03, m47;
    unpack_k4((uint32_t)h.y, (uint32_t)h.z, (uint32_t)h.w, sc03, sc47, m03, m47);
#pragma unroll
    for (int c = 0; c < 2; c++) {
      const int i = rr * 2 + c;
      r.p[i] = (float)scale_fold8(D[0][i], D[1][i], D[2][i], D[3][i], D[4][i], D[5][i], D[6][i], D[7][i], sc03, sc47);
    }
    r.dd[rr] = __fmul_rn(yd, h2f((uint16_t)((uint32_t)h.x & 0xffffu)));
    {
      int hs = __dp2a_lo((int)pw.x, (int)m03, 0);
      hs = __dp2a_hi((int)pw.y, (int)m03, hs);
      hs = __dp2a_lo((int)pw.z, (int)m47, hs);
      hs = __dp2a_hi((int)pw.w, (int)m47, hs);
      const float pmv = (float)hs, dmv = __fmul_rn(-yd, h2f((uint16_t)((uint32_t)h.x >> 16)));
      if (rr == 0) { r.pm[0] = pmv; r.ddm[0] = dmv; }
      else { r.pm[0] = (t & 1) ? pmv : r.pm[0]; r.ddm[0] = (t & 1) ? dmv : r.ddm[0]; }
    }
  }
}

template <>
__device__ __forceinline__ void block_terms<GT_Q6_K>(const uint8_t* blk, int b, const StAct& a, int lane, Terms& r) {
  const int g = lane >> 2, t = lane & 3;
  const int4* qp = (const int4*)blk;
  const int2* hp = (const int2*)(blk + 2048);
  const int4 QL[4] = {qp[lane], qp[32 + lane], qp[64 + lane], qp[96 + lane]};
  const int2 QH[4] = {hp[lane], hp[32 + lane], hp[64 + lane], hp[96 + lane]};
  const int4 s0 = ((const int4*)(blk + 3072))[g], s1 = ((const int4*)(blk + 3072))[8 + g];
  const uint16_t d0 = ((const uint16_t*)(blk + 3328))[g], d1 = ((const uint16_t*)(blk + 3328))[8 + g];
  uint32_t bA[8], bB[8];
  load_b_operands(a, b, g, t, bA, bB);
  const int4* cp = (const int4*)(a.cneg + (b * 4 + t) * 16);
  const int4 cn[4] = {cp[0], cp[1], cp[2], cp[3]};
  const int C[8][2] = {{cn[0].x, cn[0].y}, {cn[0].z, cn[0].w}, {cn[1].x, cn[1].y}, {cn[1].z, cn[1].w}, {cn[2].x, cn[2].y}, {cn[2].z, cn[2].w}, {cn[3].x, cn[3].y}, {cn[3].z, cn[3].w}};
  int D[8][4];
#pragma unroll
  for (int jj = 0; jj < 2; jj++) {
    uint32_t u[4][4];
#pragma unroll
    for (int i = 0; i < 4; i++) {
      const uint32_t A = (uint32_t)(jj ? QL[i].z : QL[i].x), B = (uint32_t)(jj ? QL[i].w : QL[i].y), H = (uint32_t)(jj ? QH[i].y : QH[i].x);
      u[0][i] = (A & 0x0f0f0f0fu) | ((H << 4) & 0x30303030u);
// ... 55 lines not shown
  for (int rr = 0; rr < 2; rr++) {
    const uint32_t a0 = sa[rr][0], a1 = sa[rr][1], a2 = sa[rr][2];
    const uint32_t w0 = __vsub4((a0 & 0x0f0f0f0fu) | ((a2 & 0x03030303u) << 4), 0x20202020u);
    const uint32_t w1 = __vsub4((a1 & 0x0f0f0f0fu) | (((a2 >> 2) & 0x03030303u) << 4), 0x20202020u);
    const uint32_t w2 = __vsub4(((a0 >> 4) & 0x0f0f0f0fu) | (((a2 >> 4) & 0x03030303u) << 4), 0x20202020u);
    const uint32_t w3 = __vsub4(((a1 >> 4) & 0x0f0f0f0fu) | (((a2 >> 6) & 0x03030303u) << 4), 0x20202020u);
    const uint32_t sel = par ? 0x7531u : 0x6420u;
    const uint32_t S0 = __byte_perm(w0, w1, sel), S1 = __byte_perm(w2, w3, sel);
#pragma unroll
    for (int c = 0; c < 2; c++) {
      const int i = rr * 2 + c;
      r.p[i] = (float)scale_fold8(D[0][i], D[1][i], D[2][i], D[3][i], D[4][i], D[5][i], D[6][i], D[7][i], S0, S1);
    }
    r.dd[rr] = __fmul_rn(yd, h2f(rr ? d1 : d0));
  }
}

template <int TYPE, bool XC>
__device__ __forceinline__ void run_item(const uint8_t* slot, uint64_t* empty_bar, int nblk, int b0, int kc, bool last, const StAct& a, int lane,
                                         volatile float* mail, volatile int* flag, const MVSeg& sg, const MVParams& p, int row0) {
  constexpr int KB = StTraits<TYPE>::KB, BB = StTraits<TYPE>::BB, NM = StTraits<TYPE>::NM;
  Terms tr[KB];
  if (nblk == KB) {
#pragma unroll
    for (int i = 0; i < KB; i++) block_terms<TYPE>(slot + i * BB, b0 + i, a, lane, tr[i]);
  } else {
#pragma unroll
    for (int i = 0; i < KB; i++) {
      if (i < nblk) block_terms<TYPE>(slot + i * BB, b0 + i, a, lane, tr[i]);
      else { Terms z{}; tr[i] = z; }
    }
  }
  __syncwarp();
  if (lane == 0) mbar_arrive(empty_bar);

  float acc[4] = {0.f, 0.f, 0.f, 0.f}, accm[2] = {0.f, 0.f};
  if (kc > 0) {
    if (lane == 0) bounded_wait([&] { return *flag >= kc; }, W_FOLD_FLAG, kc);
    __syncwarp();
    __threadfence_block();
#pragma unroll
    for (int i = 0; i < 4; i++) acc[i] = mail[i * 32 + lane];
#pragma unroll
    for (int i = 0; i < NM; i++) accm[i] = mail[(4 + i) * 32 + lane];
  }
#pragma unroll
  for (int i = 0; i < KB; i++) {
    if (i < nblk) {
#pragma unroll
      for (int q = 0; q < 4; q++) acc[q] = __fmaf_rn(tr[i].dd[q >> 1], tr[i].p[q], acc[q]);
#pragma unroll
      for (int q = 0; q < NM; q++) accm[q] = __fmaf_rn(tr[i].ddm[q], tr[i].pm[q], accm[q]);
    }
  }
  if (!last) {
    __syncwarp();
#pragma unroll
    for (int i = 0; i < 4; i++) mail[i * 32 + lane] = acc[i];
#pragma unroll
    for (int i = 0; i < NM; i++) mail[(4 + i) * 32 + lane] = accm[i];
    __threadfence_block();
    __syncwarp();
    if (lane == 0) *flag = kc + 1;
    return;
  }
  const int t = lane & 3, g = lane >> 2;
  float out[2];
#pragma unroll
  for (int rr = 0; rr < 2; rr++) {
    float u0 = acc[rr * 2], u1 = acc[rr * 2 + 1];
    u0 = __fadd_rn(u0, __shfl_xor_sync(0xffffffffu, u0, 2));
    u1 = __fadd_rn(u1, __shfl_xor_sync(0xffffffffu, u1, 2));
    u0 = __fadd_rn(u0, __shfl_xor_sync(0xffffffffu, u0, 1));
    u1 = __fadd_rn(u1, __shfl_xor_sync(0xffffffffu, u1, 1));
    float v = __fadd_rn(u0, u1);
    if (TYPE == GT_Q4_K) {
      float m = accm[rr];
      m = __fadd_rn(m, __shfl_xor_sync(0xffffffffu, m, 2));
      m = __fadd_rn(m, __shfl_xor_sync(0xffffffffu, m, 1));
      v = __fadd_rn(v, m);
    } else if (TYPE == GT_Q5_K) {
      v = __fadd_rn(v, __shfl_sync(0xffffffffu, accm[0], (lane & ~3) + rr));
    }
    out[rr] = v;
  }
  if (t < 2) {
    const int row = row0 + g + 8 * t;
    if (row < sg.w.M) {
      if (XC && a.xc) {
        const float v = epilogue(sg.epi, t ? out[1] : out[0], sg.res + row, sg.res2 + row, p);
        const XchgParams& xc = *a.xc;
        const size_t at = ((size_t)(a.epoch & 1u) * xc.world + xc.rank) * xc.n + row;
        for (int r = 0; r < xc.world; r++)
          asm volatile("st.volatile.global.v2.u32 [%0], {%1, %2};" ::"l"(xc.ll[r] + at), "r"(__float_as_uint(v)), "r"(a.epoch) : "memory");
      } else {
        store_epilogue(sg, p, row, t ? out[1] : out[0]);
      }
    }
  }
}

struct TileSpace {
  int tiles[MV_MAX_SEG], cost[MV_MAX_SEG], nseg, ntiles;
  long total;
  template <bool Q3 = true>
  __host__ __device__ __forceinline__ void init(const MVParams& p) {
    nseg = p.nseg; ntiles = 0; total = 0;
#pragma unroll
    for (int s = 0; s < MV_MAX_SEG; s++) {
      tiles[s] = s < p.nseg ? (p.seg[s].w.M + ST_ROWS - 1) / ST_ROWS : 0;
      cost[s] = s < p.nseg ? st_tile_cost<Q3>(p.seg[s].w.type) : 1;
      ntiles += tiles[s]; total += (long)tiles[s] * cost[s];
    }
  }
  __host__ __device__ __forceinline__ int locate(int& tile) const {
    static_assert(MV_MAX_SEG == 3, "locate() is written out for three segments");
    if (tile < tiles[0]) return 0;
    tile -= tiles[0];
    if (tile < tiles[1]) return 1;
    tile -= tiles[1];
    return 2;
  }
  __host__ __device__ __forceinline__ int boundary(int c, int G) const {
    if (c >= G) return ntiles;
    long target = total * c / G;
    int base = 0;
#pragma unroll
    for (int s = 0; s < MV_MAX_SEG; s++) {
      const long span = (long)tiles[s] * cost[s];
      if (target < span || s == MV_MAX_SEG - 1) return base + (int)min((long)tiles[s], (target + cost[s] / 2) / cost[s]);
      target -= span; base += tiles[s];
    }
    return ntiles;
  }
};

enum : int { PH_MATVEC = 0, PH_ATTN = 1, PH_EMBED = 2, PH_PICK = 3,
              PH_XCHG = 4 };
constexpr int XC_MAX_WORLD = 8;
struct XchgParams {
  int world, rank, index, n;
  int role;
  uint2* ll[XC_MAX_WORLD];
};
struct PickParams { const float* logits; int* state; int* out_tokens; int n; };
struct alignas(16) Phase {
  int kind;
  int q6;
  MVParams mv;
  AttnParams at;
  EmbedParams em;
  PickParams pk;
  XchgParams xc;
};

struct StepArgs {
  const Phase* prog;
  int n_phases;
  int n_slots;
  unsigned* sync;
  const int* bounds;
  unsigned long long* trace;
};

__device__ __forceinline__ unsigned ld_relaxed_u32(const unsigned* p) {
  unsigned v;
  asm volatile("ld.relaxed.gpu.global.u32 %0, [%1];" : "=r"(v) : "l"(p) : "memory");
  return v;
}
__device__ __forceinline__ unsigned ld_acquire_u32(const unsigned* p) {
  unsigned v;
  asm volatile("ld.acquire.gpu.global.u32 %0, [%1];" : "=r"(v) : "l"(p) : "memory");
  return v;
}

struct TileInfo { int seg, til, nch, type; };
template <bool Q3>
__device__ __forceinline__ TileInfo tile_info(const TileSpace& ts, const MVParams& p, int tile, int nb, bool valid) {
  TileInfo ti;
  ti.seg = 0; ti.til = 0; ti.nch = 0; ti.type = GT_Q4_K;
  if (valid) {
    int tl = tile;
    ti.seg = ts.locate(tl);
    ti.til = tl;
    ti.type = ti.seg == 0 ? p.seg[0].w.type : (ti.seg == 1 ? p.seg[1].w.type : p.seg[2].w.type);
    ti.nch = st_chunks<Q3>(ti.type, nb);
  }
  return ti;
}

struct StItem { const uint8_t* src; uint32_t bytes; };
template <bool Q3>
__device__ __forceinline__ StItem st_item(const MVParams& p, int seg, int type, int til, int kc, int nb) {
  const int kb = st_chunk_blocks<Q3>(type), bb = st_block_bytes<Q3>(type);
  const int nblk = min(kb, nb - kc * kb);
  const uint8_t* base = seg == 0 ? p.seg[0].w.st : (seg == 1 ? p.seg[1].w.st : p.seg[2].w.st);
  return {base + ((size_t)til * nb + (size_t)kc * kb) * bb, (uint32_t)(nblk * bb)};
}

struct AttnRingV { int nchv, cv, n_v; };
__host__ __device__ inline AttnRingV attn_ring_v(int T) {
  AttnRingV v;
  v.nchv = (T + 255) >> 8;
  v.cv = max(1, min(8, ST_SLOT / (v.nchv * 512)));
  v.n_v = (ATTN_CH + v.cv - 1) / v.cv;
  return v;
}
struct AttnRing : AttnPos, AttnRingV { int n_k, rpi; };
template <bool GEN>
__device__ __forceinline__ AttnRing attn_ring_geom(const AttnParams& p) {
  AttnRing g;
  static_cast<AttnPos&>(g) = attn_pos(p, p.state);
  g.rpi = ST_SLOT / ((GEN ? k_stride(p.hd) : p.hd) * 2);
  if (g.T == 0) { g.n_k = 0; g.n_v = 0; g.cv = 1; g.nchv = 0; return g; }
  static_cast<AttnRingV&>(g) = attn_ring_v(g.T);
  g.n_k = (g.pos + g.rpi - 1) / g.rpi;
  return g;
}
__device__ __forceinline__ int attn_group_ch(int hd, int cg) { return min(ATTN_CH, hd - cg * ATTN_CH); }
template <bool GEN>
__device__ __forceinline__ int attn_ring_nv(const AttnRing& g, int hd, int cg) { return GEN && g.n_v > 0 ? (attn_group_ch(hd, cg) + g.cv - 1) / g.cv : g.n_v; }

template <bool GEN>
__device__ __forceinline__ void st_attn_produce(const AttnParams& p, uint8_t* ring, uint64_t* full_bar, uint64_t* empty_bar, uint32_t S, uint32_t& seq) {
  const int lane = threadIdx.x & 31;
  const AttnRing g = attn_ring_geom<GEN>(p);
  const int n_cg = GEN ? attn_groups(p.hd) : p.hd / ATTN_CH, n_tasks = p.n_head * n_cg, group = p.n_head / p.n_kv, row_bytes = (GEN ? k_stride(p.hd) : p.hd) * 2;
  for (int task = blockIdx.x; task < n_tasks; task += gridDim.x) {
    const int h = task / n_cg, cg = task % n_cg, kvh = h / group;
    const int step = min(32, ST_W * (int)S);
    for (int i0 = 0; i0 < g.n_k; i0 += step) {
      const int i = i0 + lane;
      if (lane < step && i < g.n_k) {
        const uint32_t n = seq + (uint32_t)i;
        const RingPos rp = st_ring(n, S);
        const int rows = min(g.rpi, g.pos - i * g.rpi);
        mbar_wait(&empty_bar[rp.slot], rp.parity ^ 1u, W_FREE_K_SLOT, (int)n);
        mbar_expect_tx(&full_bar[rp.slot], (uint32_t)(rows * row_bytes));
        bulk_g2s(ring + (size_t)rp.slot * ST_SLOT, p.kc + k_row<GEN>(kvh, i * g.rpi, p.n_ctx, p.hd), (uint32_t)(rows * row_bytes), &full_bar[rp.slot]);
      }
      __syncwarp();
    }
    seq += (uint32_t)g.n_k;
    const int n_v = attn_ring_nv<GEN>(g, p.hd, cg), ch_g = GEN ? attn_group_ch(p.hd, cg) : ATTN_CH;
    for (int iv = lane; iv < n_v; iv += 32) {
      const uint32_t n = seq + (uint32_t)iv;
      const RingPos rp = st_ring(n, S);
      const int nch = min(g.cv, ch_g - iv * g.cv);
      const uint32_t bytes = (uint32_t)(g.nchv * 512);
      mbar_wait(&empty_bar[rp.slot], rp.parity ^ 1u, W_FREE_V_SLOT, (int)n);
      mbar_expect_tx(&full_bar[rp.slot], bytes * nch);
      for (int q = 0; q < nch; q++)
        bulk_g2s(ring + (size_t)rp.slot * ST_SLOT + (size_t)q * bytes, p.vc + v_chan(kvh, cg * ATTN_CH + iv * g.cv + q, p.n_ctx, p.hd), bytes,
                 &full_bar[rp.slot]);
    }
    __syncwarp();
    seq += (uint32_t)n_v;
  }
}

template <bool GEN>
__device__ __forceinline__ void st_attn_task(const AttnParams& p, uint8_t* smem, const uint8_t* ring, uint64_t* full_bar, uint64_t* empty_bar, uint32_t S, uint32_t seq0,
                                             const AttnRing& g, int h, int cg, float* red_f, double* red_d) {
  const int warp = threadIdx.x >> 5, lane = threadIdx.x & 31, nch = GEN ? attn_group_ch(p.hd, cg) : ATTN_CH;
  const AttnScratch s = attn_scratch<GEN>(smem, p.n_ctx, p.hd, true);
  attn_stage<ST_NT, GEN>(p, s, 0, h, cg, g.pos, attn_cs0<ST_NT>(p, g.pos));
  bar_sync<ST_BAR, ST_NT>();
  for (int i = (int)(((uint32_t)warp + ST_W - seq0 % ST_W) % ST_W); i < g.n_k; i += ST_W) {
    const uint32_t n = seq0 + (uint32_t)i;
    const RingPos rp = st_ring(n, S);
    const int r0 = i * g.rpi;
    mbar_wait(&full_bar[rp.slot], rp.parity, W_K_ITEM, (int)n);
    attn_scores<GEN>(p.hd, (const uint16_t*)(ring + (size_t)rp.slot * ST_SLOT), min(g.rpi, g.pos - r0), 0, 8, s.q16, p.kq_scale, s.sc + r0);
    __syncwarp();
    if (lane == 0) mbar_arrive(&empty_bar[rp.slot]);
  }
  if (warp == (int)((seq0 + (uint32_t)g.n_k) % ST_W)) attn_scores<GEN>(p.hd, s.k16, 1, 0, 8, s.q16, p.kq_scale, s.sc + g.pos);
  bar_sync<ST_BAR, ST_NT>();
  attn_softmax<ST_NT, ST_BAR>(s.sc, s.p16, g.T, p.exp_tab, red_f, red_d);
  for (int cc = warp; cc < nch; cc += ST_W) {
    const int c = cg * ATTN_CH + cc;
    const uint32_t n = seq0 + (uint32_t)(g.n_k + cc / g.cv);
    const RingPos rp = st_ring(n, S);
    mbar_wait(&full_bar[rp.slot], rp.parity, W_V_ITEM, (int)n);
    const uint16_t* vrow = (const uint16_t*)(ring + (size_t)rp.slot * ST_SLOT + (size_t)(cc % g.cv) * g.nchv * 512);
    const float o = attn_vp(vrow, s.p16, g, g.pos, s.v16[c]);
    if (lane == 0) p.out[(size_t)h * p.hd + c] = o;
  }
  bar_sync<ST_BAR, ST_NT>();
  if ((int)threadIdx.x < attn_ring_nv<GEN>(g, p.hd, cg)) {
    const uint32_t n = seq0 + (uint32_t)(g.n_k + threadIdx.x);
    mbar_arrive(&empty_bar[st_ring(n, S).slot]);
  }
}

template <bool GEN>
__device__ __forceinline__ void st_attn_phase(const Phase& ph, uint8_t* act_smem, uint8_t* ring, uint64_t* full_bar, uint64_t* empty_bar, int n_slots,
                                              uint32_t& seq, float* pick_v, double* red) {
  const int n_cg = GEN ? attn_groups(ph.at.hd) : ph.at.hd / ATTN_CH, n_tasks = ph.at.n_head * n_cg, G = (int)gridDim.x;
  if (ph.q6) {
    const AttnRing ag = attn_ring_geom<GEN>(ph.at);
    for (int task = blockIdx.x; task < n_tasks; task += G) {
      if (task != (int)blockIdx.x) bar_sync<ST_BAR, ST_NT>();
      if (ag.T > 0) st_attn_task<GEN>(ph.at, act_smem, ring, full_bar, empty_bar, (uint32_t)(n_slots / ST_W), seq, ag, task / n_cg, task % n_cg, pick_v, red);
      seq += (uint32_t)(ag.n_k + attn_ring_nv<GEN>(ag, ph.at.hd, task % n_cg));
    }
  } else {
    for (int task = blockIdx.x; task < n_tasks; task += G) {
      if (task != (int)blockIdx.x) bar_sync<ST_BAR, ST_NT>();
      attn_body<ST_NT, ST_BAR, false, GEN>(ph.at, act_smem, task / n_cg, 0, task % n_cg, ph.at.state);
    }
  }
}
template <bool Q3>
static __device__ __noinline__ uint32_t st_attn_phase_gen(const Phase& ph, uint8_t* act_smem, uint8_t* ring, uint64_t* full_bar, uint64_t* empty_bar, int n_slots,
                                                   uint32_t seq, float* pick_v, double* red) {
  st_attn_phase<true>(ph, act_smem, ring, full_bar, empty_bar, n_slots, seq, pick_v, red);
  return seq;
}

template <bool XC, bool GEN, bool Q3>
__device__ __forceinline__ void st_producer(const StepArgs& args, uint8_t* ring, uint64_t* full_bar, uint64_t* empty_bar) {
  const int lane = threadIdx.x & 31;
  const uint32_t S = (uint32_t)(args.n_slots / ST_W);
  const uint64_t weight_pol = l2_policy_evict_first();
  uint32_t seq = 0;
  for (int ip = 0; ip < args.n_phases; ip++) {
    const Phase* ph = args.prog + ip;
    if (ph->kind == PH_ATTN) {
      if (ph->q6) {
        if (GEN) st_attn_produce<true>(ph->at, ring, full_bar, empty_bar, S, seq);
        else st_attn_produce<false>(ph->at, ring, full_bar, empty_bar, S, seq);
      }
      continue;
    }
    if (ph->kind != PH_MATVEC) continue;
    const MVParams& p = ph->mv;
    TileSpace ts;
    ts.init<Q3>(p);
    const int* bnd = args.bounds + (size_t)ip * (gridDim.x + 1) + blockIdx.x;
    const int T0 = __ldg(bnd), T1 = __ldg(bnd + 1);
    const int nb = p.K >> 8;
    for (int w0 = T0; w0 < T1; w0 += ST_MAXT) {
      const int ntw = min(ST_MAXT, T1 - w0);
      const TileInfo ti = tile_info<Q3>(ts, p, w0 + lane, nb, lane < ntw);
      for (int kc = 0;; kc++) {
        const unsigned mask = __ballot_sync(0xffffffffu, kc < ti.nch);
        if (!mask) break;
        const int rank = __popc(mask & ((1u << lane) - 1u)), cnt = __popc(mask);
        for (int base = 0; base < cnt; base += ST_W * (int)S) {
          if (((mask >> lane) & 1u) && rank >= base && rank < base + ST_W * (int)S) {
            const uint32_t n = seq + (uint32_t)rank;
            const RingPos rp = st_ring(n, S);
            const StItem it = st_item<Q3>(p, ti.seg, ti.type, ti.til, kc, nb);
            mbar_wait(&empty_bar[rp.slot], rp.parity ^ 1u, W_FREE_WEIGHT_SLOT, (int)n);
            mbar_expect_tx(&full_bar[rp.slot], it.bytes);
            bulk_g2s_hint(ring + (size_t)rp.slot * ST_SLOT, it.src, it.bytes, &full_bar[rp.slot], weight_pol);
          }
          __syncwarp();
        }
        __syncwarp();
        seq += (uint32_t)__popc(mask);
      }
    }
  }
}

template <bool XC, bool Q3>
__device__ __forceinline__ void st_matvec_phase(const Phase& ph, const NormPre& np, uint8_t* ring, uint8_t* act_smem, double* red, uint64_t* full_bar, uint64_t* empty_bar,
                                                float (*mailbox)[ST_STATE * 32], int* flags, uint32_t S, uint32_t& seq, const int* tb, unsigned long long* tr,
                                                unsigned xc_base) {
  const MVParams& p = ph.mv;
  const int warp = threadIdx.x >> 5, lane = threadIdx.x & 31;
  const unsigned epoch = XC ? xc_base + (unsigned)ph.xc.index + 1u : 0u;
  stage_activation<ST_NT, ST_BAR, XC>(p, np, ACT_Q8_K, act_smem, red, blockIdx.x == 0, epoch);
  StAct a = st_act_extras<ST_NT, ST_BAR>(act_smem, p.K, ph.q6 != 0);
  a.xc = XC && ph.xc.role == 2 ? &ph.xc : nullptr;
  a.epoch = epoch;
  if (tr && threadIdx.x == 0) tr[1] = globaltimer_ns();
  bool first_item = tr != nullptr && threadIdx.x == 0;
  TileSpace ts;
  ts.init<Q3>(p);
  const int nb = p.K >> 8;
  const int T0 = tb[0], T1 = tb[1];
#pragma unroll 1
  for (int w0 = T0; w0 < T1; w0 += ST_MAXT) {
    if (w0 != T0) {
      bar_sync<ST_BAR, ST_NT>();
      if (threadIdx.x < ST_MAXT) flags[threadIdx.x] = 0;
      bar_sync<ST_BAR, ST_NT>();
    }
    const int ntw = min(ST_MAXT, T1 - w0);
    const TileInfo ti = tile_info<Q3>(ts, p, w0 + lane, nb, lane < ntw);
#pragma unroll 1
    for (int kc = 0;; kc++) {
      const unsigned mask = __ballot_sync(0xffffffffu, kc < ti.nch);
      if (!mask) break;
      const int cnt = __popc(mask);
#pragma unroll 1
      for (int r = (int)(((uint32_t)warp + ST_W - seq % ST_W) % ST_W); r < cnt; r += ST_W) {
        unsigned mr = mask;
        for (int q = 0; q < r; q++) mr &= mr - 1;
        const int j = __ffs(mr) - 1;
        const int seg = __shfl_sync(0xffffffffu, ti.seg, j), til = __shfl_sync(0xffffffffu, ti.til, j), type = __shfl_sync(0xffffffffu, ti.type, j);
        const int nch = __shfl_sync(0xffffffffu, ti.nch, j);
        const uint32_t n = seq + (uint32_t)r;
        const RingPos rp = st_ring(n, S);
        const int kb = st_chunk_blocks<Q3>(type);
        const int b0 = kc * kb, nblk = min(kb, nb - b0);
        const MVSeg& sg = p.seg[seg];
        const uint8_t* sp = ring + (size_t)rp.slot * ST_SLOT;
        mbar_wait(&full_bar[rp.slot], rp.parity, W_WEIGHT_ITEM, (int)n);
        if (first_item) { tr[2] = globaltimer_ns(); first_item = false; }
        volatile float* mail = mailbox[j];
        volatile int* flag = flags + j;
        const bool last = kc == nch - 1;
        if (type == GT_Q4_K) run_item<GT_Q4_K, XC>(sp, &empty_bar[rp.slot], nblk, b0, kc, last, a, lane, mail, flag, sg, p, til * ST_ROWS);
        else if (type == GT_Q6_K) run_item<GT_Q6_K, XC>(sp, &empty_bar[rp.slot], nblk, b0, kc, last, a, lane, mail, flag, sg, p, til * ST_ROWS);
        else if (Q3 && type == GT_Q3_K) run_item<GT_Q3_K, XC>(sp, &empty_bar[rp.slot], nblk, b0, kc, last, a, lane, mail, flag, sg, p, til * ST_ROWS);
        else run_item<GT_Q5_K, XC>(sp, &empty_bar[rp.slot], nblk, b0, kc, last, a, lane, mail, flag, sg, p, til * ST_ROWS);
      }
      seq += (uint32_t)cnt;
    }
  }
}

__device__ __forceinline__ void st_pick_phase(const PickParams& pk, float* bv, int* bi) {
  float best;
  int idx;
  block_argmax<ST_NT, ST_BAR, true>(pk.logits, pk.n, bv, bi, best, idx);
  if (threadIdx.x == 0) {
    pk.state[4] = idx;
    advance_state(pk.state, pk.out_tokens, idx);
  }
}

__device__ __forceinline__ void grid_rearm(unsigned* sync, bool set_xc = false, unsigned xc = 0) {
  if (threadIdx.x == 0) {
    __threadfence();
    if (atomicAdd(sync + 1, 1u) == gridDim.x - 1) {
      sync[0] = 0u;
      sync[1] = 0u;
      if (set_xc) sync[2] = xc;
      __threadfence();
    }
  }
}

template <bool XC, bool GEN, bool Q3>
static __global__ void __launch_bounds__(ST_THREADS, 1) k_step(const __grid_constant__ StepArgs args) {
  extern __shared__ __align__(16) uint8_t smem[];
  __shared__ __align__(8) uint64_t full_bar[ST_MAX_SLOTS];
  __shared__ __align__(8) uint64_t empty_bar[ST_MAX_SLOTS];
  __shared__ double red[3 * ST_W];
  __shared__ __align__(16) float mailbox[ST_MAXT][ST_STATE * 32];
  __shared__ int flags[ST_MAXT];
  __shared__ float pick_v[ST_W];
  __shared__ int pick_i[ST_W];
  __shared__ __align__(16) Phase ph_s[2];
  __shared__ int tb_s[2][2];
  const int warp = threadIdx.x >> 5;
  uint8_t* ring = smem;
  uint8_t* act_smem = smem + (size_t)args.n_slots * ST_SLOT;
  ring_init(full_bar, empty_bar, args.n_slots, 1);
  pdl_trigger();
  pdl_wait();
  if (warp == ST_W) {
    st_producer<XC, GEN, Q3>(args, ring, full_bar, empty_bar);
    return;
  }
  const unsigned G = gridDim.x;
  uint32_t seq = 0;
  const unsigned xc_base = XC ? ld_relaxed_u32(args.sync + 2) : 0u;
  unsigned xc_done = 0;
  auto fetch_phase = [&](int ip) {
    if (ip >= args.n_phases) return;
    const uint4* src = (const uint4*)(args.prog + ip);
    const uint32_t dst = st_smem(&ph_s[ip & 1]);
    const int i = (int)threadIdx.x - 32;
    if (i >= 0 && i < (int)(sizeof(Phase) / 16)) asm volatile("cp.async.ca.shared.global [%0], [%1], 16;" ::"r"(dst + i * 16), "l"(src + i) : "memory");
    if (i >= 64 && i < 66)
      asm volatile("cp.async.ca.shared.global [%0], [%1], 4;" ::"r"(st_smem(&tb_s[ip & 1][i - 64])), "l"(args.bounds + (size_t)ip * (gridDim.x + 1) + blockIdx.x + (i - 64)) : "memory");
    asm volatile("cp.async.commit_group;" ::: "memory");
  };
  fetch_phase(0);
#pragma unroll 1
  for (int ip = 0; ip < args.n_phases; ip++) {
    bar_sync<ST_BAR, ST_NT>();
    unsigned long long* const tr = args.trace ? args.trace + ((size_t)ip * G + blockIdx.x) * 8 : nullptr;
    if (tr && threadIdx.x == 0) tr[4] = globaltimer_ns();
    if (threadIdx.x == 0 && ip > 0) {
      const unsigned target = (unsigned)ip * G;
      asm volatile("red.release.gpu.global.add.u32 [%0], 1;" ::"l"(args.sync) : "memory");
      if (tr) tr[5] = globaltimer_ns();
      bounded_wait([&] { return ld_relaxed_u32(args.sync) >= target; }, W_GRID_BARRIER, ip);
      if (tr) { tr[6] = globaltimer_ns(); tr[7] = tr[6]; }
    } else {
      asm volatile("cp.async.wait_all;" ::: "memory");
      if (threadIdx.x >= 32 && threadIdx.x < 32 + ST_MAXT) flags[threadIdx.x - 32] = 0;
    }
    bar_sync<ST_BAR, ST_NT>();
    const Phase& ph = ph_s[ip & 1];
    fetch_phase(ip + 1);
    NormPre np;
    if (ph.kind == PH_MATVEC) preload_norm(np, ph.mv);
    if (tr && threadIdx.x == 0) tr[0] = globaltimer_ns();
    if (XC && ph.kind == PH_MATVEC && ph.xc.role == 1) xc_done++;
    if (ph.kind == PH_MATVEC) {
      st_matvec_phase<XC, Q3>(ph, np, ring, act_smem, red, full_bar, empty_bar, mailbox, flags, (uint32_t)(args.n_slots / ST_W), seq, &tb_s[ip & 1][0], tr, xc_base);
    } else if (ph.kind == PH_ATTN) {
      if (GEN) seq = st_attn_phase_gen<Q3>(ph, act_smem, ring, full_bar, empty_bar, args.n_slots, seq, pick_v, red);
      else st_attn_phase<false>(ph, act_smem, ring, full_bar, empty_bar, args.n_slots, seq, pick_v, red);
    } else if (ph.kind == PH_EMBED) {
      if (blockIdx.x == 0) embed_row<Q3>(ph.em, ph.em.tokens[0], ph.em.out, threadIdx.x, ST_NT);
    } else if (ph.kind == PH_PICK) {
      if (blockIdx.x == 0) st_pick_phase(ph.pk, pick_v, pick_i);
    }
    if (tr) {
      bar_sync<ST_BAR, ST_NT>();
      if (threadIdx.x == 0) tr[3] = globaltimer_ns();
    }
  }
  bar_sync<ST_BAR, ST_NT>();
  grid_rearm(args.sync, XC, xc_base + xc_done);
}

struct StepLaunch { int grid; int n_slots; size_t smem; bool gen = false, q3 = false;  };

inline StepLaunch step_launch_shape(const Phase* phases, int n, int n_sm, size_t max_dyn_smem, size_t extra_act = 0) {
  size_t act = extra_act;
  for (int i = 0; i < n; i++) {
    if (phases[i].kind == PH_MATVEC) act = std::max(act, st_act_bytes(phases[i].mv.K, phases[i].q6 != 0));
    if (phases[i].kind == PH_ATTN) act = std::max(act, attn_smem_bytes(phases[i].at.n_ctx, phases[i].at.hd));
  }
  bool gen = false, q3 = false;
  for (int i = 0; i < n; i++) {
    gen |= phases[i].kind == PH_ATTN && !attn_fast_hd(phases[i].at.hd);
    if (phases[i].kind == PH_MATVEC)
      for (int s = 0; s < phases[i].mv.nseg; s++) q3 |= phases[i].mv.seg[s].w.type == GT_Q3_K;
    q3 |= phases[i].kind == PH_EMBED && phases[i].em.type == GT_Q3_K;
  }
  act = (act + 127) & ~(size_t)127;
  StepLaunch L;
  L.grid = n_sm;
  L.gen = gen;
  L.q3 = q3;
  if (act + (size_t)ST_W * ST_SLOT > max_dyn_smem) { L.n_slots = 0; L.smem = 0; return L; }
  L.n_slots = ST_W * (int)std::min<size_t>(ST_MAX_DEPTH, (max_dyn_smem - act) / ((size_t)ST_W * ST_SLOT));
  L.smem = (size_t)L.n_slots * ST_SLOT + act;
  return L;
}

inline std::vector<int> step_bounds(const Phase* phs, int n, int grid) {
  std::vector<int> b((size_t)n * (grid + 1), 0);
  for (int i = 0; i < n; i++) {
    if (phs[i].kind != PH_MATVEC) continue;
    TileSpace ts;
    ts.init(phs[i].mv);
    for (int c = 0; c <= grid; c++) b[(size_t)i * (grid + 1) + c] = ts.boundary(c, grid);
  }
  return b;
}

inline bool st_attn_ring_ok(int n_ctx, int n_slots) { return attn_ring_v(n_ctx).n_v <= n_slots; }

inline bool step_supports(const MVParams& p) {
  if (p.K % 256) return false;
  for (int s = 0; s < p.nseg; s++)
    if (!type_is_kquant(p.seg[s].w.type) || !p.seg[s].w.st) return false;
  return p.nseg >= 1;
}
inline Phase matvec_phase(const MVParams& p) {
  Phase ph{};
  ph.kind = PH_MATVEC;
  ph.mv = p;
  ph.mv.act = ACT_Q8_K;
  for (int s = 0; s < p.nseg; s++) ph.q6 |= p.seg[s].w.type == GT_Q6_K || p.seg[s].w.type == GT_Q3_K;
  return ph;
}

static inline cudaError_t st_set_debug_words(int* dev_ptr) { return cudaMemcpyToSymbol(g_st_dbg, &dev_ptr, sizeof(int*)); }
static inline cudaError_t step_set_smem_limit(size_t bytes) {
  void (*const kernels[])(StepArgs) = {k_step<false, false, false>, k_step<false, true, false>, k_step<true, false, false>,
                                        k_step<false, false, true>, k_step<false, true, true>, k_step<true, false, true>};
  for (auto k : kernels) {
    const cudaError_t e = cudaFuncSetAttribute(k, cudaFuncAttributeMaxDynamicSharedMemorySize, (int)bytes);
    if (e != cudaSuccess) return e;
  }
  return cudaSuccess;
}

static inline cudaError_t launch_step(const StepLaunch& L, cudaStream_t st, const Phase* d_prog, const int* d_bounds, int n_phases, unsigned* d_sync, bool pdl = false,
                                      unsigned long long* trace = nullptr, bool xchg = false) {
  StepArgs a;
  a.prog = d_prog; a.bounds = d_bounds; a.n_phases = n_phases; a.n_slots = L.n_slots; a.sync = d_sync; a.trace = trace;
  auto kernel = L.q3 ? (xchg ? k_step<true, false, true> : (L.gen ? k_step<false, true, true> : k_step<false, false, true>))
                     : (xchg ? k_step<true, false, false> : (L.gen ? k_step<false, true, false> : k_step<false, false, false>));
  return launch_kernel(kernel, dim3(L.grid), dim3(ST_THREADS), L.smem, st, pdl, a);
}

}
```

ctransformers_b200/lib.py:

```python
import ctypes as C
from pathlib import Path
from typing import Optional

LIB_DIR = Path(__file__).resolve().parent / "lib"
LIB_NAME = "libctransformers.so"


class ConfigStruct(C.Structure):
    _fields_ = [("context_length", C.c_int), ("gpu_layers", C.c_int), ("mmap", C.c_bool), ("mlock", C.c_bool)]


def find_library(path: Optional[str] = None) -> str:
    if path:
        return str(path)
    lib = LIB_DIR / LIB_NAME
    if not lib.is_file():
        raise OSError(
            f"{lib} has not been built. Build it with `python -m ctransformers_b200.build` "
            "(needs nvcc; compiles for sm_90a). There is no CPU fallback library."
        )
    return str(lib)


_P = C.c_void_p
_IP = C.POINTER(C.c_int)
_FP = C.POINTER(C.c_float)
_DP = C.POINTER(C.c_double)

PROTOTYPES = {
    "ctransformers_llm_create": (_P, [C.c_char_p, C.c_char_p, ConfigStruct]),
    "ctransformers_llm_delete": (None, [_P]),
    "ctransformers_llm_tokenize": (C.c_int, [_P, C.c_char_p, C.c_bool, _IP]),
    "ctransformers_llm_detokenize": (C.c_char_p, [_P, C.c_int]),
    "ctransformers_llm_is_eos_token": (C.c_bool, [_P, C.c_int]),
    "ctransformers_llm_eos_token_id": (C.c_int, [_P]),
    "ctransformers_llm_bos_token_id": (C.c_int, [_P]),
    "ctransformers_llm_vocab_size": (C.c_int, [_P]),
    "ctransformers_llm_context_length": (C.c_int, [_P]),
    "ctransformers_llm_architecture": (C.c_char_p, [_P]),
    "ctransformers_llm_batch_eval": (C.c_bool, [_P, _IP, C.c_int, C.c_int, C.c_int, C.c_int]),
    "ctransformers_llm_logits_data": (_FP, [_P]),
    "ctransformers_llm_logits_size": (C.c_int, [_P]),
    "ctransformers_llm_embeddings_data": (_FP, [_P]),
    "ctransformers_llm_embeddings_size": (C.c_int, [_P]),
    "ctransformers_llm_sample": (C.c_int, [_P, _IP, C.c_int, C.c_int, C.c_float, C.c_float, C.c_float, C.c_int]),
    "ctransformers_llm_reset": (None, [_P]),
}
EXTRA_PROTOTYPES = {
    "ctb_abi_version": (C.c_int, []),
    "ctb_llm_last_eval_ms": (C.c_double, [_P]),
    "ctb_llm_launches_per_token": (C.c_long, [_P]),
    "ctb_llm_speculative_hits": (C.c_long, [_P]),
    "ctb_llm_weight_bytes_per_token": (C.c_ulonglong, [_P]),
    "ctb_llm_trace_step": (C.c_long, [_P, C.c_int, C.c_int, C.POINTER(C.c_ulonglong), C.c_long]),
    "ctb_llm_load_ms": (C.c_double, [_P]),
    "ctb_llm_device_samples": (C.c_long, [_P]),
    "ctb_llm_set_stream": (None, [_P, C.c_void_p]),
    "ctb_tp_unique_id": (C.c_int, [_P, C.c_int]),
    "ctb_llm_create_tp": (_P, [C.c_char_p, C.c_char_p, ConfigStruct, C.c_int, C.c_int, _P]),
    "ctb_tp_shard": (C.c_int, [C.c_int, C.c_int, C.c_int, C.c_int, C.c_int, C.c_int, _IP]),
    "ctb_llm_decode_greedy": (C.c_double, [_P, C.c_int, C.c_int, C.c_int, _IP]),
    "ctb_llm_profile_step": (C.c_int, [_P, C.c_int, C.c_int, C.POINTER(C.c_double), _IP]),
    "ctb_llm_time_matvec_only": (C.c_double, [_P, C.c_int, C.POINTER(C.c_long)]),
    "ctb_llm_time_matvec_kinds": (C.c_double, [_P, C.c_int, C.POINTER(C.c_long), C.c_uint]),
    "ctb_mul_mat": (C.c_int, [C.c_int, _P, _P, _P, C.c_int, C.c_int, C.c_int]),
    "ctb_quantize_row_q8_K": (C.c_int, [_P, _P, C.c_int]),
    "ctb_quantize_row_q8_0": (C.c_int, [_P, _P, C.c_int]),
    "ctb_quantize_row_q8_1": (C.c_int, [_P, _P, C.c_int]),
    "ctb_norm": (C.c_int, [C.c_int, _P, _P, _P, _P, C.c_int, C.c_float]),
    "ctb_norm_path": (C.c_int, [C.c_int, C.c_int, _P, _P, _P, _P, C.c_int, C.c_float]),
    "ctb_rope": (C.c_int, [_P, C.c_int, C.c_int, C.c_int, C.c_int, C.c_float, C.c_float]),
    "ctb_attention": (C.c_int, [_P, _P, _P, _P, C.c_int, C.c_int, C.c_int, C.c_int, C.c_int, C.c_float]),
    "ctb_attention_path": (C.c_int, [C.c_int, _P, _P, _P, _P, _P, _P, C.c_int, C.c_int, C.c_int, C.c_int, C.c_int, C.c_int, _P, C.c_int,
                                     C.c_float, C.c_float]),
    "ctb_prefill_mul_mat": (C.c_int, [C.c_int, _P, _P, _P, C.c_int, C.c_int, _P, _P, C.c_int, _P, _P, C.c_float, _P, _P, _P, _P, C.c_int,
                                      C.c_int, _P]),
    "ctb_llm_paths": (C.c_long, [_P, _IP, C.c_int]),
    "ctb_ffn_gate": (C.c_int, [C.c_int, _P, _P, _P, _P, C.c_int, C.c_int]),
    "ctb_matvec_partition": (C.c_int, [_IP, _IP, C.c_int, C.c_int, C.c_int, _IP, _IP]),
    "ctb_get_row": (C.c_int, [C.c_int, _P, C.c_int, C.c_int, C.c_int, _P]),
    "ctb_argmax_path": (C.c_int, [C.c_int, _P, C.c_int, _IP]),
    "ctb_sample_topk": (C.c_int, [_P, C.c_int, _IP, C.c_int, C.c_float, C.c_int, _IP, _P]),
    "ctb_sample_device": (C.c_int, [_P, C.c_int, _IP, C.c_int, C.c_int, C.c_float, C.c_float, C.c_float, C.c_int, _IP]),
    "ctb_sample_topk_rows": (C.c_int, [_P, C.c_int, C.c_int, _IP, _IP, _FP, _IP, _IP, _IP, _FP]),
    "ctb_sample_device_rows": (C.c_int, [_P, C.c_int, C.c_int, _IP, _IP, _IP, _FP, _FP, _FP, _IP, _IP, _IP]),
    "ctb_vocab_load": (_P, [C.c_char_p]),
    "ctb_vocab_free": (None, [_P]),
    "ctb_vocab_size": (C.c_int, [_P]),
    "ctb_vocab_tokenize": (C.c_int, [_P, C.c_char_p, C.c_bool, _IP, C.c_int]),
    "ctb_vocab_piece": (C.c_int, [_P, C.c_int, C.c_char_p, C.c_int]),
    "ctb_sample": (C.c_int, [_FP, C.c_int, _IP, C.c_int, C.c_int, C.c_float, C.c_float, C.c_float, C.c_int]),
    "ctb_multi_create": (_P, [C.c_char_p, C.c_char_p, ConfigStruct, C.c_int]),
    "ctb_multi_delete": (None, [_P]),
    "ctb_multi_info": (C.c_int, [_P, _IP]),
    "ctb_multi_eval": (C.c_bool, [_P, C.c_int, _IP, _IP, _IP, _IP, C.c_int]),
    "ctb_multi_logits": (_FP, [_P, C.c_int]),
    "ctb_multi_embeddings": (_FP, [_P, C.c_int]),
    "ctb_multi_greedy": (C.c_int, [_P, C.c_int, _IP, _IP]),
    "ctb_multi_sample": (C.c_int, [_P, C.c_int, _IP, C.c_int, C.c_int, C.c_float, C.c_float, C.c_float, C.c_int]),
    "ctb_multi_sample_many": (C.c_int, [_P, C.c_int, _IP, _IP, _IP, _IP, _FP, _FP, _FP, _IP, _IP]),
    "ctb_multi_device_samples": (C.c_long, [_P]),
    "ctb_multi_reset": (C.c_int, [_P, C.c_int]),
    "ctb_multi_launches": (C.c_long, [_P]),
    "ctb_multi_last_eval_ms": (C.c_double, [_P]),
    "ctb_multi_pack": (C.c_int, [C.c_int, _IP, _IP, _IP, C.c_int, C.c_int, _IP, C.c_int]),
    "ctb_state_info": (C.c_int, [_P, C.c_size_t, _P]),
    "ctb_llm_state_size": (C.c_size_t, [_P, C.c_int]),
    "ctb_llm_save_state": (C.c_int, [_P, _IP, C.c_int, _P, C.c_size_t]),
    "ctb_llm_load_state": (C.c_int, [_P, _P, C.c_size_t]),
    "ctb_multi_state_size": (C.c_size_t, [_P, C.c_int]),
    "ctb_multi_save": (C.c_int, [_P, C.c_int, _IP, C.c_int, _P, C.c_size_t]),
    "ctb_multi_restore": (C.c_int, [_P, C.c_int, _P, C.c_size_t]),
    "ctb_multi_fork": (C.c_int, [_P, C.c_int, C.c_int, _IP]),
    "ctb_llm_batch_eval_rows": (C.c_int, [_P, _IP, C.c_int, C.c_int, C.c_int, _FP]),
    "ctb_llm_batch_eval_scored": (C.c_int, [_P, _IP, C.c_int, C.c_int, C.c_int, _IP, _DP, _IP]),
    "ctb_llm_score_last": (C.c_int, [_P, C.c_int, _DP, _IP]),
    "ctb_row_logprob": (C.c_int, [_P, C.c_int, C.c_int, _IP, _DP, _IP]),
    "ctb_multi_eval_rows": (C.c_int, [_P, C.c_int, _IP, _IP, _IP, _IP, C.c_int, _FP]),
    "ctb_multi_eval_scored": (C.c_int, [_P, C.c_int, _IP, _IP, _IP, _IP, C.c_int, _IP, _DP, _IP]),
    "ctb_beam_step": (C.c_int, [C.c_int, C.c_int, C.c_int, _FP, _P, _FP, C.c_int, _IP, _IP, _FP, _P]),
    "ctb_multi_reparent": (C.c_long, [_P, C.c_int, _IP, _IP, _IP, _IP]),
    "ctb_multi_beam_search": (C.c_int, [_P, C.c_int, _IP, _IP, C.c_int, C.c_int, C.c_int, _IP, _IP, _FP]),
    "ctb_multi_beam_stats": (C.c_int, [_P, _DP]),
}


class StateHeader(C.Structure):
    _fields_ = [("magic", C.c_uint32), ("version", C.c_uint32), ("n_layer", C.c_int32), ("n_head_kv", C.c_int32), ("head_dim", C.c_int32),
                ("k_stride", C.c_int32), ("n_embd", C.c_int32), ("n_vocab", C.c_int32), ("n_tokens", C.c_int32), ("has_results", C.c_int32),
                ("fingerprint", C.c_uint64)]


def load_library(path: Optional[str] = None):
    lib = C.CDLL(find_library(path))
    for table, required in ((PROTOTYPES, True), (EXTRA_PROTOTYPES, False)):
        for name, (res, args) in table.items():
            try:
                fn = getattr(lib, name)
            except AttributeError:
                if required:
                    raise OSError(f"{path or LIB_NAME} does not export '{name}'")
                continue
            fn.restype, fn.argtypes = res, args
    return lib
```

include/ctransformers_b200.h:

```cpp
#ifndef CTRANSFORMERS_B200_H_
#define CTRANSFORMERS_B200_H_

#include <stdbool.h>
#include <stddef.h>
#include <stdint.h>

#ifdef __cplusplus
extern "C" {
#endif

typedef struct LLM LLM;

typedef struct ctransformers_config {
  int context_length;
  int gpu_layers;
  bool mmap;
  bool mlock;
} ctransformers_config;

LLM* ctransformers_llm_create(const char* model_path, const char* model_type, const ctransformers_config config);
void ctransformers_llm_delete(LLM* llm);
int ctransformers_llm_tokenize(LLM* llm, const char* text, const bool add_bos_token, int* output);
const char* ctransformers_llm_detokenize(LLM* llm, const int token);
bool ctransformers_llm_is_eos_token(LLM* llm, const int token);
int ctransformers_llm_eos_token_id(LLM* llm);
int ctransformers_llm_bos_token_id(LLM* llm);
int ctransformers_llm_vocab_size(LLM* llm);
int ctransformers_llm_context_length(LLM* llm);
const char* ctransformers_llm_architecture(LLM* llm);
bool ctransformers_llm_batch_eval(LLM* llm, const int* tokens, const int n_tokens, const int n_past, const int batch_size,
                                  const int threads);
float* ctransformers_llm_logits_data(LLM* llm);
int ctransformers_llm_logits_size(LLM* llm);
const float* ctransformers_llm_embeddings_data(LLM* llm);
int ctransformers_llm_embeddings_size(LLM* llm);
int ctransformers_llm_sample(LLM* llm, const int* last_tokens, const int n_last, const int top_k, const float top_p,
                             const float temperature, const float repetition_penalty, int seed);
void ctransformers_llm_reset(LLM* llm);

int ctb_abi_version(void);
double ctb_llm_last_eval_ms(LLM* llm);
long ctb_llm_launches_per_token(LLM* llm);
long ctb_llm_speculative_hits(LLM* llm);
unsigned long long ctb_llm_weight_bytes_per_token(LLM* llm);
long ctb_llm_device_samples(LLM* llm);
double ctb_llm_load_ms(LLM* llm);
int ctb_tp_unique_id(void* out, int cap);
LLM* ctb_llm_create_tp(const char* model_path, const char* model_type, const ctransformers_config config, int rank, int world,
                       const void* unique_id);
int ctb_tp_shard(int n_embd, int n_head, int n_head_kv, int n_ff, int rank, int world, int* out6);
void ctb_llm_set_stream(LLM* llm, void* cuda_stream);
double ctb_llm_decode_greedy(LLM* llm, int first_token, int n_past, int n_steps, int* out_tokens);

int ctb_llm_profile_step(LLM* llm, int token, int n_past, double* ms_by_kind, int* count_by_kind);
long ctb_llm_trace_step(LLM* llm, int token, int n_past, unsigned long long* out, long cap_words);
double ctb_llm_time_matvec_only(LLM* llm, int reps, long* launches);
double ctb_llm_time_matvec_kinds(LLM* llm, int reps, long* launches, unsigned kind_mask);
long ctb_llm_paths(LLM* llm, int* out, int cap);

typedef struct ctb_vocab ctb_vocab;
ctb_vocab* ctb_vocab_load(const char* gguf_path);
void ctb_vocab_free(ctb_vocab* v);
int ctb_vocab_size(ctb_vocab* v);
int ctb_vocab_tokenize(ctb_vocab* v, const char* text, bool add_bos, int* out, int cap);
int ctb_vocab_piece(ctb_vocab* v, int token, char* buf, int cap);
int ctb_sample(const float* logits, int n_vocab, const int* last_tokens, int n_last, int top_k, float top_p, float temperature,
               float repetition_penalty, int seed);

int ctb_mul_mat(int type, const void* w_blocks, const float* x, float* dst, int K, int M, int N);
int ctb_quantize_row_q8_K(const float* x, void* y, int k);
int ctb_quantize_row_q8_0(const float* x, void* y, int k);
int ctb_quantize_row_q8_1(const float* x, void* y, int k);
int ctb_norm(int mode, const float* x, const float* w, const float* b, float* y, int n, float eps);
int ctb_norm_path(int path, int mode, const float* x, const float* w, const float* b, float* y, int n, float eps);
int ctb_rope(float* x, int n_heads, int head_dim, int pos, int mode, float freq_base, float freq_scale);
int ctb_attention(const float* q, const uint16_t* kcache, const uint16_t* vcache, float* out, int n_head, int n_kv, int head_dim,
                  int T, int n_total, float kq_scale);
int ctb_attention_path(int path, const float* q, const float* k_new, const float* v_new, uint16_t* kcache, uint16_t* vcache,
                       float* out, int n_head, int n_kv, int head_dim, int n_ctx, int pos0, int n_tok, const int* n_total,
                       int rope_mode, float freq_base, float kq_scale);
int ctb_prefill_mul_mat(int nseg, const int* types, const void* const* w_blocks, const int* rows, int K, int n_tok, const float* x,
                        const float* x2, int norm_mode, const float* norm_w, const float* norm_b, float eps, const int* epi,
                        const float* res, const float* res2, float* out, int n_ctx, int head_dim, int* n_slots);
int ctb_ffn_gate(int type, const void* w1_blocks, const void* w3_blocks, const float* x, float* out, int K, int M);
int ctb_matvec_partition(const int* types, const int* rows, int nseg, int K, int n_sm, int* first_tile, int* meta);

int ctb_get_row(int type, const void* table_blocks, int K, int n_rows, int row, float* out);

int ctb_argmax_path(int path, const float* logits, int n, int* out);
int ctb_sample_topk(const float* logits, int n, const int* last_tokens, int n_last, float repetition_penalty, int k, int* ids, float* lg);
int ctb_sample_device(const float* logits, int n, const int* last_tokens, int n_last, int top_k, float top_p, float temperature,
                      float repetition_penalty, int seed, int* used_device);
int ctb_sample_topk_rows(const float* logits, int n_rows, int n, const int* last_off, const int* last_tokens, const float* repetition_penalty,
                         const int* k, int* count, int* ids, float* lg);
int ctb_sample_device_rows(const float* logits, int n_rows, int n, const int* last_off, const int* last_tokens, const int* top_k, const float* top_p,
                           const float* temperature, const float* repetition_penalty, const int* seed, int* tokens, int* used_device);

typedef struct ctb_multi ctb_multi;
ctb_multi* ctb_multi_create(const char* model_path, const char* model_type, const ctransformers_config config, int n_slots);
void ctb_multi_delete(ctb_multi* m);
int ctb_multi_info(ctb_multi* m, int* out6);
bool ctb_multi_eval(ctb_multi* m, int n, const int* slots, const int* off, const int* tokens, const int* n_past, int batch_size);
const float* ctb_multi_logits(ctb_multi* m, int slot);
const float* ctb_multi_embeddings(ctb_multi* m, int slot);
int ctb_multi_greedy(ctb_multi* m, int n, const int* slots, int* out);
int ctb_multi_sample(ctb_multi* m, int slot, const int* last_tokens, int n_last, int top_k, float top_p, float temperature,
                     float repetition_penalty, int seed);
int ctb_multi_sample_many(ctb_multi* m, int n, const int* slots, const int* last_off, const int* last_tokens, const int* top_k, const float* top_p,
                          const float* temperature, const float* repetition_penalty, const int* seed, int* out);
long ctb_multi_device_samples(ctb_multi* m);
int ctb_multi_reset(ctb_multi* m, int slot);
long ctb_multi_launches(ctb_multi* m);
double ctb_multi_last_eval_ms(ctb_multi* m);
int ctb_multi_pack(int n, const int* slots, const int* off, const int* n_past, int batch_size, int n_ctx, int* out, int cap);

#define CTB_STATE_MAGIC 0x53425443u
#define CTB_STATE_VERSION 1u
typedef struct ctb_state_header {
  uint32_t magic, version;
  int32_t n_layer, n_head_kv, head_dim, k_stride, n_embd, n_vocab;
  int32_t n_tokens;
  int32_t has_results;
  uint64_t fingerprint;
} ctb_state_header;
int ctb_state_info(const void* buf, size_t size, ctb_state_header* out);
size_t ctb_llm_state_size(LLM* llm, int n_tokens);
int ctb_llm_save_state(LLM* llm, const int* tokens, int n_tokens, void* buf, size_t cap);
int ctb_llm_load_state(LLM* llm, const void* buf, size_t size);
size_t ctb_multi_state_size(ctb_multi* m, int n_tokens);
int ctb_multi_save(ctb_multi* m, int slot, const int* tokens, int n_tokens, void* buf, size_t cap);
int ctb_multi_restore(ctb_multi* m, int slot, const void* buf, size_t size);
int ctb_multi_fork(ctb_multi* m, int src, int n, const int* dsts);

int ctb_multi_beam_search(ctb_multi* m, int n_prompts, const int* prompt_off, const int* prompt_tokens, int n_beams, int n_predict, int batch_size,
                          int* out_off, int* out_tokens, float* out_p);
int ctb_multi_beam_stats(ctb_multi* m, double* out8);
int ctb_beam_step(int n_beams, int n_in, int n_next, const float* in_p, const unsigned char* in_eob, const float* rows, int n_vocab, int* out_parent,
                  int* out_token, float* out_p, unsigned char* out_eob);
long ctb_multi_reparent(ctb_multi* m, int n, const int* src, const int* dst, const int* lo, const int* hi);

int ctb_llm_batch_eval_rows(LLM* llm, const int* tokens, int n_tokens, int n_past, int batch_size, float* rows);
int ctb_llm_batch_eval_scored(LLM* llm, const int* tokens, int n_tokens, int n_past, int batch_size, const int* targets, double* logprob,
                              int* greedy);
int ctb_llm_score_last(LLM* llm, int target, double* logprob, int* greedy);
int ctb_row_logprob(const float* rows, int n_rows, int n_vocab, const int* targets, double* logprob, int* greedy);
int ctb_multi_eval_rows(ctb_multi* m, int n, const int* slots, const int* off, const int* tokens, const int* n_past, int batch_size, float* rows);
int ctb_multi_eval_scored(ctb_multi* m, int n, const int* slots, const int* off, const int* tokens, const int* n_past, int batch_size,
                          const int* targets, double* logprob, int* greedy);

#ifdef __cplusplus
}
#endif
#endif
```

Baseline: 364.2.

## Replace grid barriers with per-block readiness counters between dependent step phases

Adds a dataflow hand-off between adjacent fused phases: producers (attention tasks or matvec tiles) publish per-256-element-block completion counters, and the consuming matvec waits only on the blocks it is about to quantize instead of the whole-grid barrier. Consumer activation staging is rewritten to quantize block by block after each block is ready, and the counters are reset by the last CTA at kernel end. This aims to remove the full grid barrier stall between phases such as attention to wo and w2 to the next op, at the cost of extra atomics, per-block waits and more complex memory ordering.

```diff
diff --git a/ctransformers_b200/csrc/engine.cu b/ctransformers_b200/csrc/engine.cu
--- a/ctransformers_b200/csrc/engine.cu
+++ b/ctransformers_b200/csrc/engine.cu
@@ -643,15 +643,63 @@
   if (any_stream && step_slots_ < ST_W) throw std::runtime_error("model rows are too long for the step kernel's shared memory");
   if (any_stream) CTB_CUDA(step_set_smem_limit(step_smem_));
   else fused_ = false;
+  plan_handoff();
   d_prog_ = (Phase*)alloc((ops_.size() + 1) * sizeof(Phase), 256);
   d_prog_mv_ = (Phase*)alloc((ops_.size() + 1) * sizeof(Phase), 256);
   d_bounds_ = (int*)alloc((ops_.size() + 1) * (size_t)(sm_count_ + 1) * 4, 256);
   d_bounds_mv_ = (int*)alloc((ops_.size() + 1) * (size_t)(sm_count_ + 1) * 4, 256);
 }
 
+void Engine::plan_handoff() {
+  n_ready_ = 0;
+  const char* off = getenv("CTB_NO_HANDOFF");
+  if (!fused_ || tp_.world > 1 || (off && off[0] == '1')) return;
+  auto writes = [](const Phase& ph, const float* buf) {
+    if (ph.kind == PH_ATTN) return buf == ph.at.out;
+    for (int s = 0; s < ph.mv.nseg; s++) if (ph.mv.seg[s].out == buf) return true;
+    return buf == ph.mv.norm_out;
+  };
+  auto pair_ok = [&](const StepOp& pr, const StepOp& c) {
+    const MVParams& q = c.ph.mv;
+    if (c.ph.kind != PH_MATVEC || !c.stream || q.norm_mode != NORM_NONE || (q.x_mode != 0 && q.x_mode != 1)) return false;
+    for (int s = 0; s < q.nseg; s++)
+      if ((pr.ph.kind == PH_ATTN && (q.seg[s].out == pr.ph.at.q || q.seg[s].out == pr.ph.at.k || q.seg[s].out == pr.ph.at.v)) ||
+          (pr.ph.kind == PH_MATVEC && (q.seg[s].out == pr.ph.mv.x || q.seg[s].out == pr.ph.mv.x2)))
+        return false;
+    for (int s = 0; s < q.nseg; s++)
+      if ((q.seg[s].res && writes(pr.ph, q.seg[s].res)) || (q.seg[s].res2 && writes(pr.ph, q.seg[s].res2))) return false;
+    if (pr.ph.kind == PH_ATTN) return q.x_mode == 0 && q.x == pr.ph.at.out;
+    if (pr.ph.kind != PH_MATVEC || !pr.stream || pr.ph.mv.norm_out || pr.ph.mv.sum_out || pr.ph.mv.nseg != (q.x_mode == 1 ? 2 : 1)) return false;
+    for (int s = 0; s < pr.ph.mv.nseg; s++)
+      if (pr.ph.mv.seg[s].w.M != q.K || pr.ph.mv.seg[s].out != (s == 0 ? q.x : q.x2)) return false;
+    return true;
+  };
+  std::vector<unsigned> need;
+  std::vector<std::pair<size_t, size_t>> at;
+  for (size_t i = 1; i < ops_.size(); i++) {
+    if (!pair_ok(ops_[i - 1], ops_[i])) continue;
+    const std::vector<unsigned> nd = handoff_need(ops_[i - 1].ph, ops_[i].ph.mv.K);
+    at.push_back({i, need.size()});
+    need.insert(need.end(), nd.begin(), nd.end());
+  }
+  if (need.empty()) return;
+  n_ready_ = (int)need.size();
+  handoff_ = DevMem(need.size() * 8);
+  unsigned* ready = handoff_.as<unsigned>();
+  CTB_CUDA(cudaMemset(ready, 0, need.size() * 4));
+  CTB_CUDA(cudaMemcpy(ready + n_ready_, need.data(), need.size() * 4, cudaMemcpyHostToDevice));
+  for (const auto& a : at) {
+    ops_[a.first - 1].ph.ready_out = ready + a.second;
+    ops_[a.first].ph.ready_in = ready + a.second;
+    ops_[a.first].ph.need = ready + n_ready_ + a.second;
+  }
+}
+
 void Engine::upload_prog(Phase* dst, int* dst_bounds, const std::vector<StepOp>& ops) {
   std::vector<Phase> phs(ops.size());
   for (size_t i = 0; i < ops.size(); i++) phs[i] = ops[i].ph;
+  for (size_t i = 0; i < phs.size(); i++)
+    if (phs[i].ready_in && !(i > 0 && phs[i - 1].ready_out == phs[i].ready_in)) phs[i].ready_in = nullptr;
   CTB_CUDA(cudaMemcpy(dst, phs.data(), phs.size() * sizeof(Phase), cudaMemcpyHostToDevice));
   std::vector<Phase> run = phs;
   for (size_t i = 0; i < ops.size(); i++) if (ops[i].ph.kind == PH_XCHG || (ops[i].ph.kind == PH_MATVEC && !ops[i].stream)) run[i].kind = -1;
@@ -675,6 +723,7 @@
   StepLaunch step_shape_;
   step_shape_.grid = step_grid_; step_shape_.n_slots = step_slots_; step_shape_.smem = step_smem_; step_shape_.gen = !attn_fast_hd(hp_.head_dim());
   step_shape_.q3 = step_q3_;
+  step_shape_.ready = handoff_.as<unsigned>(); step_shape_.n_ready = n_ready_;
   auto capable = [&](const StepOp& op) { return op.ph.kind != PH_XCHG && (op.ph.kind != PH_MATVEC || op.stream); };
   int i = 0;
   while (i < n) {
@@ -790,6 +839,7 @@
   CTB_CUDA(cudaMemset(buf.get(), 0, (size_t)n * step_grid_ * 64));
   StepLaunch L;
   L.grid = step_grid_; L.n_slots = step_slots_; L.smem = step_smem_; L.gen = !attn_fast_hd(hp_.head_dim()); L.q3 = step_q3_;
+  L.ready = handoff_.as<unsigned>(); L.n_ready = n_ready_;
   for (int rep = 0; rep < 3; rep++) {
     put_step(token, n_past, n_past + 1);
     CTB_CUDA(launch_step(L, stream_, d_prog_, d_bounds_, n, d_sync_, false, buf.as<unsigned long long>()));
diff --git a/ctransformers_b200/csrc/engine.cuh b/ctransformers_b200/csrc/engine.cuh
--- a/ctransformers_b200/csrc/engine.cuh
+++ b/ctransformers_b200/csrc/engine.cuh
@@ -160,6 +160,9 @@
   size_t step_smem_ = 0;
   bool fused_ = true;
   bool step_q3_ = false;
+  DevMem handoff_;
+  int n_ready_ = 0;
+  void plan_handoff();
   bool ring_attn_ = false;
   void build_ops();
   void push_matvec(struct MVParams& p, int kind);
diff --git a/ctransformers_b200/csrc/matvec.cuh b/ctransformers_b200/csrc/matvec.cuh
--- a/ctransformers_b200/csrc/matvec.cuh
+++ b/ctransformers_b200/csrc/matvec.cuh
@@ -23,12 +23,13 @@
 #endif
 enum WaitCode : int {
   W_GRID_BARRIER = 1, W_FOLD_FLAG, W_FREE_WEIGHT_SLOT, W_WEIGHT_ITEM, W_FREE_K_SLOT, W_FREE_V_SLOT, W_K_ITEM, W_V_ITEM, W_XCHG,
-  W_PF_GRID_BARRIER, W_PF_FREE_SLOT, W_PF_WEIGHT_ITEM, W_CODES
+  W_PF_GRID_BARRIER, W_PF_FREE_SLOT, W_PF_WEIGHT_ITEM, W_HANDOFF_BLOCK, W_CODES
 };
 constexpr const char* WAIT_TEXT[] = {"?", "grid barrier (aux = phase)", "fold hand-off flag (aux = chunk)", "producer: free weight slot (aux = item)",
                                      "consumer: weight item (aux = item)", "producer: free K slot (attention)", "producer: free V slot (attention)",
                                      "consumer: K item (attention)", "consumer: V item (attention)", "tensor-parallel exchange: a peer's element (aux = exchange number)",
-                                     "prefill grid barrier (aux = phase)", "prefill producer: free slot (aux = item)", "prefill consumer: weight item (aux = item)"};
+                                     "prefill grid barrier (aux = phase)", "prefill producer: free slot (aux = item)", "prefill consumer: weight item (aux = item)",
+                                     "hand-off: the producing phase's tiles or tasks of an input block (aux = block)"};
 static_assert(sizeof(WAIT_TEXT) / sizeof(WAIT_TEXT[0]) == W_CODES, "one text per wait code");
 
 static __device__ int* g_st_dbg = nullptr;
@@ -189,6 +190,44 @@
     load16<true>(xs.x2 + base, valid, u);
 #pragma unroll
     for (int e = 0; e < 16; e++) v[e] = __fmul_rn(v[e], u[e]);
+  }
+}
+
+__device__ __forceinline__ void quant_q8k16(const float (&v)[16], int base, int valid, int lane, int8_t* qs, float* dd, int16_t* bs) {
+  float amax = 0.f, mx = 0.f;
+#pragma unroll
+  for (int e = 0; e < 16; e++) { const float ax = fabsf(v[e]); if (ax > amax) { amax = ax; mx = v[e]; } }
+  float gmax = amax;
+#pragma unroll
+  for (int o = 8; o > 0; o >>= 1) gmax = fmaxf(gmax, __shfl_xor_sync(0xffffffffu, gmax, o));
+  const unsigned who = __ballot_sync(0xffffffffu, amax == gmax);
+  const int hbase = lane & 16, hl = lane & 15;
+  const unsigned mine = (who >> hbase) & 0xffffu;
+  const float maxv = __shfl_sync(0xffffffffu, mx, hbase + __ffs(mine) - 1);
+  if (valid > 0) {
+    const int b = base >> 8;
+    int q[16];
+    int sum = 0;
+    if (gmax == 0.f) {
+#pragma unroll
+      for (int e = 0; e < 16; e++) q[e] = 0;
+      if (hl == 0) dd[b] = 0.f;
+    } else {
+      const float iscale = __fdiv_rn(-128.f, maxv);
+#pragma unroll
+      for (int e = 0; e < 16; e++) {
+        const float val = __fmaf_rn(iscale, v[e], 12582912.f);
+        q[e] = min(127, (__float_as_int(val) & 0x007fffff) - 0x00400000);
+        sum += q[e];
+      }
+      if (hl == 0) dd[b] = __fdiv_rn(1.f, iscale);
+    }
+    bs[b * 16 + hl] = (int16_t)sum;
+#pragma unroll
+    for (int j = 0; j < 4; j++) {
+      const int wi = hl * 4 + j;
+      *(uint32_t*)(qs + q8k_word_offset(b, wi >> 3, wi & 7)) = pack4(q + 4 * j);
+    }
   }
 }
 
@@ -340,41 +379,7 @@
       for (int e = 0; e < 16; e++) if (e < valid) norm_out[base + e] = v[e];
     }
     if (act == ACT_Q8_K) {
-      float amax = 0.f, mx = 0.f;
-#pragma unroll
-      for (int e = 0; e < 16; e++) { const float ax = fabsf(v[e]); if (ax > amax) { amax = ax; mx = v[e]; } }
-      float gmax = amax;
-#pragma unroll
-      for (int o = 8; o > 0; o >>= 1) gmax = fmaxf(gmax, __shfl_xor_sync(0xffffffffu, gmax, o));
-      const unsigned who = __ballot_sync(0xffffffffu, amax == gmax);
-      const int hbase = lane & 16, hl = lane & 15;
-      const unsigned mine = (who >> hbase) & 0xffffu;
-      const float maxv = __shfl_sync(0xffffffffu, mx, hbase + __ffs(mine) - 1);
-      if (valid > 0) {
-        const int b = base >> 8;
-        int q[16];
-        int sum = 0;
-        if (gmax == 0.f) {
-#pragma unroll
-          for (int e = 0; e < 16; e++) q[e] = 0;
-          if (hl == 0) dd[b] = 0.f;
-        } else {
-          const float iscale = __fdiv_rn(-128.f, maxv);
-#pragma unroll
-          for (int e = 0; e < 16; e++) {
-            const float val = __fmaf_rn(iscale, v[e], 12582912.f);
-            q[e] = min(127, (__float_as_int(val) & 0x007fffff) - 0x00400000);
-            sum += q[e];
-          }
-          if (hl == 0) dd[b] = __fdiv_rn(1.f, iscale);
-        }
-        bs[b * 16 + hl] = (int16_t)sum;
-#pragma unroll
-        for (int j = 0; j < 4; j++) {
-          const int wi = hl * 4 + j;
-          *(uint32_t*)(qs + q8k_word_offset(b, wi >> 3, wi & 7)) = pack4(q + 4 * j);
-        }
-      }
+      quant_q8k16(v, base, valid, lane, qs, dd, bs);
     } else if (act == ACT_Q8_0) {
       float amax = 0.f;
 #pragma unroll
diff --git a/ctransformers_b200/csrc/ops_abi.cu b/ctransformers_b200/csrc/ops_abi.cu
--- a/ctransformers_b200/csrc/ops_abi.cu
+++ b/ctransformers_b200/csrc/ops_abi.cu
@@ -608,6 +608,27 @@
   return 0;
 }
 
+int ctb_handoff_plan(int producer, const int* types, int nseg, int K, int n_head, int hd, unsigned* need) {
+  if (K <= 0) return -1;
+  Phase ph{};
+  if (producer == 1) {
+    if (n_head < 1 || hd < 1 || n_head * hd != K) return -1;
+    ph.kind = PH_ATTN; ph.at.n_head = n_head; ph.at.hd = hd;
+  } else if (producer == 0) {
+    if (nseg < 1 || nseg > MV_MAX_SEG) return -1;
+    ph.kind = PH_MATVEC; ph.mv.K = 256; ph.mv.nseg = nseg;
+    for (int s = 0; s < nseg; s++) {
+      if (!type_is_kquant(types[s])) return -1;
+      ph.mv.seg[s].w.type = types[s]; ph.mv.seg[s].w.K = 256; ph.mv.seg[s].w.M = K; ph.mv.seg[s].w.nb = 1;
+    }
+  } else {
+    return -1;
+  }
+  const std::vector<unsigned> nd = handoff_need(ph, K);
+  std::copy(nd.begin(), nd.end(), need);
+  return 0;
+}
+
 int ctb_get_row(int type, const void* table_blocks, int K, int n_rows, int row, float* out) {
   return guarded("ctb_get_row", [&] {
     const size_t rb = raw_row_bytes(type, K);
diff --git a/ctransformers_b200/csrc/stream.cuh b/ctransformers_b200/csrc/stream.cuh
--- a/ctransformers_b200/csrc/stream.cuh
+++ b/ctransformers_b200/csrc/stream.cuh
@@ -163,19 +163,27 @@
   unsigned epoch;
 };
 __host__ __device__ inline size_t st_off_pairs(int K) { return ((((size_t)K + 15) & ~(size_t)15) + q8k_d_bytes(K) + (size_t)(K / 16) * 2 + 15) & ~(size_t)15; }
-__host__ __device__ inline size_t st_act_bytes(int K, bool q6) { return st_off_pairs(K) + (size_t)(K / 256) * 16 + (q6 ? (size_t)K : 0) + 256 + 16; }
+__host__ __device__ inline size_t st_off_zero(int K, bool q6) { return st_off_pairs(K) + (size_t)(K / 256) * 16 + (q6 ? (size_t)K : 0); }
+__host__ __device__ inline size_t st_act_bytes(int K, bool q6) { return st_off_zero(K, q6) + 256 + 16; }
+
+__device__ __forceinline__ StAct st_act_view(uint8_t* smem, int K, bool q6) {
+  const ActView a = act_view(ACT_Q8_K, K, smem);
+  StAct s;
+  s.qs = a.qs; s.d = a.d;
+  s.pairs = (const uint32_t*)(smem + st_off_pairs(K));
+  s.cneg = (const int*)(smem + st_off_pairs(K) + (size_t)(K / 256) * 16);
+  s.zero = (const int8_t*)(smem + st_off_zero(K, q6));
+  return s;
+}
 
 template <int NT, int BAR>
 __device__ __forceinline__ StAct st_act_extras(uint8_t* smem, int K, bool q6) {
   const ActView a = act_view(ACT_Q8_K, K, smem);
-  StAct s;
-  s.qs = a.qs; s.d = a.d;
-  uint32_t* pairs = (uint32_t*)(smem + st_off_pairs(K));
-  int* cneg = (int*)(smem + st_off_pairs(K) + (size_t)(K / 256) * 16);
-  s.pairs = pairs; s.cneg = cneg;
+  const StAct s = st_act_view(smem, K, q6);
+  uint32_t* pairs = (uint32_t*)s.pairs;
+  int* cneg = (int*)s.cneg;
   const int nb = K >> 8;
-  int* zero = (int*)(smem + st_off_pairs(K) + (size_t)nb * 16 + (q6 ? (size_t)K : 0));
-  s.zero = (const int8_t*)zero;
+  int* zero = (int*)s.zero;
   if (threadIdx.x < 64) zero[threadIdx.x] = 0;
   for (int i = threadIdx.x; i < nb * 4; i += NT) {
     const int16_t* b4 = a.bs + (i >> 2) * 16 + 4 * (i & 3);
@@ -537,7 +545,11 @@
   EmbedParams em;
   PickParams pk;
   XchgParams xc;
+  unsigned* ready_out;
+  unsigned* ready_in;
+  const unsigned* need;
 };
+static_assert(sizeof(Phase) <= 64 * 16, "k_step fetches a phase descriptor with 64 threads of 16 bytes");
 
 struct StepArgs {
   const Phase* prog;
@@ -545,6 +557,8 @@
   int n_slots;
   unsigned* sync;
   const int* bounds;
+  unsigned* ready;
+  int n_ready;
   unsigned long long* trace;
 };
 
@@ -680,6 +694,14 @@
 }
 
 template <bool GEN>
+__device__ __forceinline__ void st_attn_publish(const Phase& ph, int h, int cg) {
+  bar_sync<ST_BAR, ST_NT>();
+  if (threadIdx.x == 0) {
+    const int c0 = h * ph.at.hd + cg * ATTN_CH, c1 = c0 + (GEN ? attn_group_ch(ph.at.hd, cg) : ATTN_CH) - 1;
+    for (int b = c0 >> 8; b <= c1 >> 8; b++) asm volatile("red.release.gpu.global.add.u32 [%0], 1;" ::"l"(ph.ready_out + b) : "memory");
+  }
+}
+template <bool GEN>
 __device__ __forceinline__ void st_attn_phase(const Phase& ph, uint8_t* act_smem, uint8_t* ring, uint64_t* full_bar, uint64_t* empty_bar, int n_slots,
                                               uint32_t& seq, float* pick_v, double* red) {
   const int n_cg = GEN ? attn_groups(ph.at.hd) : ph.at.hd / ATTN_CH, n_tasks = ph.at.n_head * n_cg, G = (int)gridDim.x;
@@ -689,11 +711,13 @@
       if (task != (int)blockIdx.x) bar_sync<ST_BAR, ST_NT>();
       if (ag.T > 0) st_attn_task<GEN>(ph.at, act_smem, ring, full_bar, empty_bar, (uint32_t)(n_slots / ST_W), seq, ag, task / n_cg, task % n_cg, pick_v, red);
       seq += (uint32_t)(ag.n_k + attn_ring_nv<GEN>(ag, ph.at.hd, task % n_cg));
+      if (ph.ready_out) st_attn_publish<GEN>(ph, task / n_cg, task % n_cg);
     }
   } else {
     for (int task = blockIdx.x; task < n_tasks; task += G) {
       if (task != (int)blockIdx.x) bar_sync<ST_BAR, ST_NT>();
       attn_body<ST_NT, ST_BAR, false, GEN>(ph.at, act_smem, task / n_cg, 0, task % n_cg, ph.at.state);
+      if (ph.ready_out) st_attn_publish<GEN>(ph, task / n_cg, task % n_cg);
     }
   }
 }
@@ -751,15 +775,58 @@
   }
 }
 
+__device__ __forceinline__ StAct st_stage_handoff(const Phase& ph, uint8_t* act_smem) {
+  const MVParams& p = ph.mv;
+  const int warp = threadIdx.x >> 5, lane = threadIdx.x & 31, hl = lane & 15, nb = p.K >> 8;
+  const bool q6 = ph.q6 != 0;
+  const StAct a = st_act_view(act_smem, p.K, q6);
+  const ActView av = act_view(ACT_Q8_K, p.K, act_smem);
+  if (threadIdx.x < 64) ((int*)a.zero)[threadIdx.x] = 0;
+#pragma unroll 1
+  for (int pr = warp; 2 * pr < nb; pr += ST_W) {
+    const int b = 2 * pr + (lane >> 4), valid = b < nb ? 16 : 0;
+    if (valid && hl == 0) bounded_wait([&] { return ld_acquire_u32(ph.ready_in + b) >= __ldg(ph.need + b); }, W_HANDOFF_BLOCK, b);
+    __syncwarp();
+    const int base = min(b, nb - 1) * 256 + hl * 16;
+    float v[16];
+    load16x(p, base, valid, v);
+    quant_q8k16(v, base, valid, lane, (int8_t*)av.qs, (float*)av.d, (int16_t*)av.bs);
+    __syncwarp();
+    if (valid) {
+      if (hl < 4) {
+        const int16_t* b4 = av.bs + b * 16 + 4 * hl;
+        const int p0 = (int)b4[0] + (int)b4[1], p1 = (int)b4[2] + (int)b4[3];
+        ((uint32_t*)a.pairs)[b * 4 + hl] = (uint32_t)(p0 & 0xffff) | ((uint32_t)p1 << 16);
+      }
+      if (q6) {
+#pragma unroll
+        for (int j = 0; j < 4; j++) {
+          const int i = hl * 4 + j, grp = i >> 3, l = i & 7;
+          const int w = *(const int*)(av.qs + q8k_word_offset(b, grp, l));
+          ((int*)a.cneg)[((b * 4 + (l >> 1)) * 8 + grp) * 2 + (l & 1)] = -32 * __dp4a(0x01010101, w, 0);
+        }
+      }
+    }
+  }
+  bar_sync<ST_BAR, ST_NT>();
+  return a;
+}
+
 template <bool XC, bool Q3>
 __device__ __forceinline__ void st_matvec_phase(const Phase& ph, const NormPre& np, uint8_t* ring, uint8_t* act_smem, double* red, uint64_t* full_bar, uint64_t* empty_bar,
                                                 float (*mailbox)[ST_STATE * 32], int* flags, uint32_t S, uint32_t& seq, const int* tb, unsigned long long* tr,
-                                                unsigned xc_base) {
+                                                unsigned xc_base, bool handoff) {
   const MVParams& p = ph.mv;
   const int warp = threadIdx.x >> 5, lane = threadIdx.x & 31;
   const unsigned epoch = XC ? xc_base + (unsigned)ph.xc.index + 1u : 0u;
-  stage_activation<ST_NT, ST_BAR, XC>(p, np, ACT_Q8_K, act_smem, red, blockIdx.x == 0, epoch);
-  StAct a = st_act_extras<ST_NT, ST_BAR>(act_smem, p.K, ph.q6 != 0);
+  const bool consumer = !XC && handoff;
+  StAct a;
+  if (consumer) {
+    a = st_stage_handoff(ph, act_smem);
+  } else {
+    stage_activation<ST_NT, ST_BAR, XC>(p, np, ACT_Q8_K, act_smem, red, blockIdx.x == 0, epoch);
+    a = st_act_extras<ST_NT, ST_BAR>(act_smem, p.K, ph.q6 != 0);
+  }
   a.xc = XC && ph.xc.role == 2 ? &ph.xc : nullptr;
   a.epoch = epoch;
   if (tr && threadIdx.x == 0) tr[1] = globaltimer_ns();
@@ -820,7 +887,7 @@
   }
 }
 
-__device__ __forceinline__ void grid_rearm(unsigned* sync, bool set_xc = false, unsigned xc = 0) {
+__device__ __forceinline__ bool grid_rearm(unsigned* sync, bool set_xc = false, unsigned xc = 0) {
   if (threadIdx.x == 0) {
     __threadfence();
     if (atomicAdd(sync + 1, 1u) == gridDim.x - 1) {
@@ -828,7 +895,28 @@
       sync[1] = 0u;
       if (set_xc) sync[2] = xc;
       __threadfence();
-    }
+      return true;
+    }
+  }
+  return false;
+}
+
+template <bool Q3>
+__device__ __forceinline__ void st_publish_tiles(const Phase& ph, int T0, int T1) {
+  TileSpace ts;
+  ts.init<Q3>(ph.mv);
+  asm volatile("fence.acq_rel.gpu;" ::: "memory");
+  int blk = -1, cnt = 0;
+  for (int tile = T0; tile <= T1; tile++) {
+    int b = -1;
+    if (tile < T1) {
+      int tl = tile;
+      ts.locate(tl);
+      b = tl * ST_ROWS / 256;
+    }
+    if (b != blk && cnt) asm volatile("red.relaxed.gpu.global.add.u32 [%0], %1;" ::"l"(ph.ready_out + blk), "r"(cnt) : "memory");
+    if (b != blk) { blk = b; cnt = 0; }
+    cnt++;
   }
 }
 
@@ -844,6 +932,7 @@
   __shared__ int pick_i[ST_W];
   __shared__ __align__(16) Phase ph_s[2];
   __shared__ int tb_s[2][2];
+  __shared__ int last_cta;
   const int warp = threadIdx.x >> 5;
   uint8_t* ring = smem;
   uint8_t* act_smem = smem + (size_t)args.n_slots * ST_SLOT;
@@ -869,13 +958,19 @@
     asm volatile("cp.async.commit_group;" ::: "memory");
   };
   fetch_phase(0);
+  unsigned long long next_in = 0;
+  unsigned n_bar = 0;
 #pragma unroll 1
   for (int ip = 0; ip < args.n_phases; ip++) {
     bar_sync<ST_BAR, ST_NT>();
     unsigned long long* const tr = args.trace ? args.trace + ((size_t)ip * G + blockIdx.x) * 8 : nullptr;
     if (tr && threadIdx.x == 0) tr[4] = globaltimer_ns();
-    if (threadIdx.x == 0 && ip > 0) {
-      const unsigned target = (unsigned)ip * G;
+    if (!XC && threadIdx.x == 0 && ip > 0) {
+      const Phase& pp = ph_s[(ip - 1) & 1];
+      if (pp.kind == PH_MATVEC && pp.ready_out) st_publish_tiles<Q3>(pp, tb_s[(ip - 1) & 1][0], tb_s[(ip - 1) & 1][1]);
+    }
+    if (threadIdx.x == 0 && ip > 0 && (XC || !next_in)) {
+      const unsigned target = ++n_bar * G;
       asm volatile("red.release.gpu.global.add.u32 [%0], 1;" ::"l"(args.sync) : "memory");
       if (tr) tr[5] = globaltimer_ns();
       bounded_wait([&] { return ld_relaxed_u32(args.sync) >= target; }, W_GRID_BARRIER, ip);
@@ -887,12 +982,14 @@
     bar_sync<ST_BAR, ST_NT>();
     const Phase& ph = ph_s[ip & 1];
     fetch_phase(ip + 1);
+    if (!XC && threadIdx.x == 0 && ip + 1 < args.n_phases) next_in = __ldg((const unsigned long long*)&args.prog[ip + 1].ready_in);
     NormPre np;
     if (ph.kind == PH_MATVEC) preload_norm(np, ph.mv);
     if (tr && threadIdx.x == 0) tr[0] = globaltimer_ns();
     if (XC && ph.kind == PH_MATVEC && ph.xc.role == 1) xc_done++;
     if (ph.kind == PH_MATVEC) {
-      st_matvec_phase<XC, Q3>(ph, np, ring, act_smem, red, full_bar, empty_bar, mailbox, flags, (uint32_t)(args.n_slots / ST_W), seq, &tb_s[ip & 1][0], tr, xc_base);
+      st_matvec_phase<XC, Q3>(ph, np, ring, act_smem, red, full_bar, empty_bar, mailbox, flags, (uint32_t)(args.n_slots / ST_W), seq, &tb_s[ip & 1][0], tr, xc_base,
+                              ip > 0 && ph.ready_in != nullptr);
     } else if (ph.kind == PH_ATTN) {
       if (GEN) seq = st_attn_phase_gen<Q3>(ph, act_smem, ring, full_bar, empty_bar, args.n_slots, seq, pick_v, red);
       else st_attn_phase<false>(ph, act_smem, ring, full_bar, empty_bar, args.n_slots, seq, pick_v, red);
@@ -907,10 +1004,19 @@
     }
   }
   bar_sync<ST_BAR, ST_NT>();
-  grid_rearm(args.sync, XC, xc_base + xc_done);
-}
-
-struct StepLaunch { int grid; int n_slots; size_t smem; bool gen = false, q3 = false;  };
+  const bool last = grid_rearm(args.sync, XC, xc_base + xc_done);
+  if (!XC && args.n_ready) {
+    if (threadIdx.x == 0) last_cta = last;
+    bar_sync<ST_BAR, ST_NT>();
+    if (last_cta)
+      for (int i = threadIdx.x; i < args.n_ready; i += ST_NT) args.ready[i] = 0u;
+  }
+}
+
+struct StepLaunch {
+  int grid; int n_slots; size_t smem; bool gen = false, q3 = false;
+  unsigned* ready = nullptr; int n_ready = 0;
+};
 
 inline StepLaunch step_launch_shape(const Phase* phases, int n, int n_sm, size_t max_dyn_smem, size_t extra_act = 0) {
   size_t act = extra_act;
@@ -947,6 +1053,27 @@
   return b;
 }
 
+inline std::vector<unsigned> handoff_need(const Phase& producer, int K) {
+  std::vector<unsigned> need((size_t)(K + 255) / 256, 0u);
+  if (producer.kind == PH_MATVEC) {
+    TileSpace ts;
+    ts.init(producer.mv);
+    for (int tile = 0; tile < ts.ntiles; tile++) {
+      int tl = tile;
+      ts.locate(tl);
+      need[(size_t)tl * ST_ROWS / 256]++;
+    }
+  } else if (producer.kind == PH_ATTN) {
+    const int hd = producer.at.hd, n_cg = attn_groups(hd);
+    for (int h = 0; h < producer.at.n_head; h++)
+      for (int cg = 0; cg < n_cg; cg++) {
+        const int c0 = h * hd + cg * ATTN_CH, c1 = c0 + std::min(ATTN_CH, hd - cg * ATTN_CH) - 1;
+        for (int b = c0 >> 8; b <= c1 >> 8; b++) need[b]++;
+      }
+  }
+  return need;
+}
+
 inline bool st_attn_ring_ok(int n_ctx, int n_slots) { return attn_ring_v(n_ctx).n_v <= n_slots; }
 
 inline bool step_supports(const MVParams& p) {
@@ -979,6 +1106,7 @@
                                       unsigned long long* trace = nullptr, bool xchg = false) {
   StepArgs a;
   a.prog = d_prog; a.bounds = d_bounds; a.n_phases = n_phases; a.n_slots = L.n_slots; a.sync = d_sync; a.trace = trace;
+  a.ready = L.ready; a.n_ready = L.n_ready;
   auto kernel = L.q3 ? (xchg ? k_step<true, false, true> : (L.gen ? k_step<false, true, true> : k_step<false, false, true>))
                      : (xchg ? k_step<true, false, false> : (L.gen ? k_step<false, true, false> : k_step<false, false, false>));
   return launch_kernel(kernel, dim3(L.grid), dim3(ST_THREADS), L.smem, st, pdl, a);
diff --git a/ctransformers_b200/lib.py b/ctransformers_b200/lib.py
--- a/ctransformers_b200/lib.py
+++ b/ctransformers_b200/lib.py
@@ -78,6 +78,7 @@
     "ctb_llm_paths": (C.c_long, [_P, _IP, C.c_int]),
     "ctb_ffn_gate": (C.c_int, [C.c_int, _P, _P, _P, _P, C.c_int, C.c_int]),
     "ctb_matvec_partition": (C.c_int, [_IP, _IP, C.c_int, C.c_int, C.c_int, _IP, _IP]),
+    "ctb_handoff_plan": (C.c_int, [C.c_int, _IP, C.c_int, C.c_int, C.c_int, C.c_int, C.c_void_p]),
     "ctb_get_row": (C.c_int, [C.c_int, _P, C.c_int, C.c_int, C.c_int, _P]),
     "ctb_argmax_path": (C.c_int, [C.c_int, _P, C.c_int, _IP]),
     "ctb_sample_topk": (C.c_int, [_P, C.c_int, _IP, C.c_int, C.c_float, C.c_int, _IP, _P]),
diff --git a/include/ctransformers_b200.h b/include/ctransformers_b200.h
--- a/include/ctransformers_b200.h
+++ b/include/ctransformers_b200.h
@@ -84,6 +84,7 @@
                         const float* res, const float* res2, float* out, int n_ctx, int head_dim, int* n_slots);
 int ctb_ffn_gate(int type, const void* w1_blocks, const void* w3_blocks, const float* x, float* out, int K, int M);
 int ctb_matvec_partition(const int* types, const int* rows, int nseg, int K, int n_sm, int* first_tile, int* meta);
+int ctb_handoff_plan(int producer, const int* types, int nseg, int K, int n_head, int hd, unsigned* need);
 
 int ctb_get_row(int type, const void* table_blocks, int K, int n_rows, int row, float* out);
 
```

New measurement: 366.0, median of 6. No clear change (+0.5%).
